# sp-uhh/sgmse

Measured on AMD Instinct MI355X. Metric: utterances/sec, SGMSE+ NCSN++ PC N=30 (reverse_diffusion + ALD, 60 NFE), 16 kHz 4 s utterances, higher is better.
Workload: dtype f32 (fp16x2-split products, fp32 accumulate); 1 GPU; BASELINE configs[1]: ncsnpp (65.6M params) PC sampler N=30, batch=32 x 4 s @16 kHz per GPU, hipGraph-captured step; batch_per_gpu=32, F=256, T=512, nfe=60, sampler=pc, parallelism=utterance-sharded x1 (weights broadcast once over RCCL)

## Files before the change

### sgmse_amd/csrc/conv_launch.h

```cpp
#pragma once
#include "kernels_conv.h"
#include "kernels_conv_pipe.h"
#include "kernels_conv1x1.h"
#include "kernels_conv_split.h"
#include "kernels_conv_wino.h"
#include "kernels_conv_wino2d.h"
#include "kernels_conv_thin.h"

#ifndef SGMSE_CONV_SPLIT_DEFAULT
#define SGMSE_CONV_SPLIT_DEFAULT 2
#endif
#ifndef SGMSE_CONV_PIPE_DEFAULT
#define SGMSE_CONV_PIPE_DEFAULT 1
#endif

namespace sgmse {

inline int conv_variant() {
  static int v = [] { const char* e = getenv("SGMSE_CONV_VARIANT"); return e ? atoi(e) : 0; }();
  return v;
}

inline int conv_grid_tiles(const ConvArgs& a, int rows) {
  const int ty = (a.H + rows - 1) / rows;
  return a.rag_cols ? ty * a.rag_ncols : a.B * ty * ((a.W + 31) / 32);
}

template <int KS, int WC, int FC, int FP>
inline void launch_conv_mfma_t(const ConvArgs& a, drt::stream_t st, int variant, int ksplit = 1) {
  using T = ConvTile<KS, WC, FC, FP>;
  const int tiles = conv_grid_tiles(a, T::ROWS);
  dim3 grid(tiles, (a.Cout + T::CO_T - 1) / T::CO_T, ksplit);
  if (variant < 0) variant = conv_variant();
  const bool vec = (a.rag_w ? a.rag_vec_ok != 0 : a.W % 4 == 0) && !(variant & 2) && (reinterpret_cast<uintptr_t>(a.src1) % 16 == 0) &&
                   (a.src2 == nullptr || reinterpret_cast<uintptr_t>(a.src2) % 16 == 0);
  const bool pref = !(variant & 1);
  if constexpr (FC * FP == 8) {
    const bool pipe = ((variant & 4) != 0) != (SGMSE_CONV_PIPE_DEFAULT != 0);
    if (vec && pipe) { DRT_LAUNCH((conv_mfma_pipe_kernel<KS, WC, FC, FP>), grid, dim3(256), st, a); return; }
  }
  if constexpr (KS == 1 && FC * FP == 8) {
    if (!vec) { launch_conv_mfma_t<KS, WC, FC, FP / 2>(a, st, variant, ksplit); return; }
    if (pref) DRT_LAUNCH((conv_mfma_kernel<KS, WC, FC, FP, 1, 1>), grid, dim3(256), st, a);
    else DRT_LAUNCH((conv_mfma_kernel<KS, WC, FC, FP, 0, 1>), grid, dim3(256), st, a);
  } else {
    if (vec && pref) DRT_LAUNCH((conv_mfma_kernel<KS, WC, FC, FP, 1, 1>), grid, dim3(256), st, a);
    else if (vec) DRT_LAUNCH((conv_mfma_kernel<KS, WC, FC, FP, 0, 1>), grid, dim3(256), st, a);
    else if (pref) DRT_LAUNCH((conv_mfma_kernel<KS, WC, FC, FP, 1, 0>), grid, dim3(256), st, a);
    else DRT_LAUNCH((conv_mfma_kernel<KS, WC, FC, FP, 0, 0>), grid, dim3(256), st, a);
  }
  if constexpr (FC * FP <= 2) {
    if (ksplit > 1) DRT_LAUNCH((conv_splitk_reduce_kernel<KS, WC, FC, FP>), dim3(grid.x, grid.y, 1), dim3(256), st, a, ksplit);
  }
}

inline void launch_conv_mfma(const ConvArgs& a, int ks, const ConvPlan& pl, drt::stream_t st, int variant = -1, int ksplit = 1) {
  const int v = variant < 0 ? conv_variant() : variant;
  if (ks == 1 && pl.co_t == 128 && (v & 8)) {
    const int kc = (v & 16) ? 64 : 32;
    const int Cin = a.C1 + a.C2;
    if (Cin % kc == 0 && (a.src2 == nullptr || a.C1 % kc == 0)) {
      const int tiles = conv_grid_tiles(a, 4);
      dim3 grid(tiles, a.Cout / 128, 1);
      if (kc == 64) DRT_LAUNCH((conv1x1_stream_kernel<1, 64>), grid, dim3(256), st, a);
      else DRT_LAUNCH((conv1x1_stream_kernel<1, 32>), grid, dim3(256), st, a);
      return;
    }
  }
#define SGMSE_CONV_CASE(KS_, CO_, ROWS_, WC_, FC_, FP_) \
  if (ks == KS_ && pl.co_t == CO_ && pl.rows == ROWS_) { launch_conv_mfma_t<KS_, WC_, FC_, FP_>(a, st, variant, ksplit); return; }
  SGMSE_CONV_CASE(3, 128, 8, 2, 2, 4)
  SGMSE_CONV_CASE(3, 64, 8, 2, 1, 4)
  SGMSE_CONV_CASE(3, 32, 8, 1, 1, 2)
  SGMSE_CONV_CASE(3, 128, 4, 2, 2, 2)
  SGMSE_CONV_CASE(3, 64, 4, 2, 1, 2)
  SGMSE_CONV_CASE(3, 32, 4, 1, 1, 1)
  SGMSE_CONV_CASE(1, 128, 8, 2, 2, 4)
  SGMSE_CONV_CASE(1, 64, 8, 2, 1, 4)
  SGMSE_CONV_CASE(1, 32, 8, 1, 1, 2)
  SGMSE_CONV_CASE(1, 128, 4, 2, 2, 2)
  SGMSE_CONV_CASE(1, 64, 4, 2, 1, 2)
  SGMSE_CONV_CASE(1, 32, 4, 1, 1, 1)
#undef SGMSE_CONV_CASE
}

inline bool conv_split_eligible(int ks, int C1, int C2, int Cout) {
  return (ks == 3 || ks == 1) && Cout % 128 == 0 && (C1 + C2) % 16 == 0 && (C2 == 0 || C1 % 16 == 0) && (C1 + C2) <= 512;
}
inline bool conv_thin_split_eligible(int ks, int C1, int C2, int Cout) {
  return ks == 3 && Cout <= 32 && (C1 + C2) >= 64 && (C1 + C2) % 16 == 0 && (C2 == 0 || C1 % 16 == 0) && (C1 + C2) <= 512;
}
template <class S, int SHAPE>
inline void launch_conv3x3_split_t(const ConvArgs& a, dim3 grid, drt::stream_t st) {
  const bool act = a.in_scale && a.in_act;
  if constexpr (SHAPE != 1 && S::SCALED) {
    if (a.sc_w) {
      DRT_LAUNCH((conv3x3_split_kernel<S, SHAPE, 1, 0, 1>), grid, dim3(256), st, a);
      return;
    }
  }
  if (act) DRT_LAUNCH((conv3x3_split_kernel<S, SHAPE, 1>), grid, dim3(256), st, a);
  else DRT_LAUNCH((conv3x3_split_kernel<S, SHAPE, 0>), grid, dim3(256), st, a);
}
inline int conv_split_stats_rows(int ks, int Cout) { return (ks == 3 && Cout <= 32) ? 1 : 4; }
inline void launch_conv_split(const ConvArgs& a, int ks, int mode, drt::stream_t st, bool rows4 = false, int abl = 0, int ksplit = 1) {
  const int tiles = conv_grid_tiles(a, 8);
  if (ks == 3 && a.Cout > 32 && rows4 && a.kchunk_stages > 0 && mode == 2) {
    const dim3 grid(conv_grid_tiles(a, 4), a.Cout / 128, ksplit);
    if (a.in_scale && a.in_act) DRT_LAUNCH((conv3x3_split_kernel<SplitH2, 2, 1, 0, 0, 1>), grid, dim3(256), st, a);
    else DRT_LAUNCH((conv3x3_split_kernel<SplitH2, 2, 0, 0, 0, 1>), grid, dim3(256), st, a);
    if (ksplit > 1) DRT_LAUNCH((conv_splitk_reduce_kernel<3, 4, 1, 4, true>), dim3(grid.x, grid.y, 1), dim3(256), st, a, ksplit);
    return;
  }
  if (ks == 3 && a.Cout > 32 && rows4) {
    const dim3 grid(conv_grid_tiles(a, 4), a.Cout / 128, 1);
    if (mode == 2) launch_conv3x3_split_t<SplitH2, 2>(a, grid, st); else launch_conv3x3_split_t<SplitB3, 2>(a, grid, st);
    return;
  }
  if (ks == 3 && a.Cout <= 32) {
    if (mode == 2) launch_conv3x3_split_t<SplitH2, 1>(a, dim3(tiles, 1, 1), st); else launch_conv3x3_split_t<SplitB3, 1>(a, dim3(tiles, 1, 1), st);
    return;
  }
  if (ks == 1) {
    if (mode == 2) DRT_LAUNCH(conv1x1_split_kernel<SplitH2>, dim3(tiles, a.Cout / 128, 1), dim3(256), st, a);
    else DRT_LAUNCH(conv1x1_split_kernel<SplitB3>, dim3(tiles, a.Cout / 128, 1), dim3(256), st, a);
    return;
  }
  const dim3 grid(tiles, a.Cout / 128, 1);
  if (abl && mode == 2) {
#define SGMSE_ABL_CASE(V) if (abl == V) { DRT_LAUNCH((conv3x3_split_kernel<SplitH2, 0, 1, V>), grid, dim3(256), st, a); return; }
#ifdef SGMSE_ABLATION_FULL
    SGMSE_ABL_CASE(8) SGMSE_ABL_CASE(59) SGMSE_ABL_CASE(64)
    SGMSE_ABL_CASE(3) SGMSE_ABL_CASE(4) SGMSE_ABL_CASE(24) SGMSE_ABL_CASE(56)
    SGMSE_ABL_CASE(1) SGMSE_ABL_CASE(2) SGMSE_ABL_CASE(67) SGMSE_ABL_CASE(72) SGMSE_ABL_CASE(128) SGMSE_ABL_CASE(256) SGMSE_ABL_CASE(512)
#endif
#undef SGMSE_ABL_CASE
  }
  if (mode == 2) launch_conv3x3_split_t<SplitH2, 0>(a, grid, st); else launch_conv3x3_split_t<SplitB3, 0>(a, grid, st);
}

inline bool conv_wino_eligible(int C1, int C2, int Cout, int W) {
  return Cout % 128 == 0 && (C1 + C2) % 16 == 0 && (C2 == 0 || C1 % 16 == 0) && (C1 + C2) <= 512 && W % 2 == 0;
}
inline void launch_conv_wino(const ConvArgs& a, drt::stream_t st, bool rows4, bool trace = false, int abl = 0) {
  const bool act = a.in_scale && a.in_act;
#ifdef SGMSE_ABLATION_FULL
#define SGMSE_WABL_CASE(V) if (abl == V) { DRT_LAUNCH((conv3x3_wino_kernel<8, 1, 0, 0, V>), dim3(conv_grid_tiles(a, 8), a.Cout / 128, 1), dim3(512), st, a); return; }
  SGMSE_WABL_CASE(1) SGMSE_WABL_CASE(2) SGMSE_WABL_CASE(4) SGMSE_WABL_CASE(8) SGMSE_WABL_CASE(16) SGMSE_WABL_CASE(24) SGMSE_WABL_CASE(3) SGMSE_WABL_CASE(32) SGMSE_WABL_CASE(20)
#undef SGMSE_WABL_CASE
  if (trace) { DRT_LAUNCH((conv3x3_wino_kernel<8, 1, 0, 1>), dim3(conv_grid_tiles(a, 8), a.Cout / 128, 1), dim3(512), st, a); return; }
#endif
  (void)abl; (void)trace;
  if (rows4) {
    const dim3 grid(conv_grid_tiles(a, 4), a.Cout / 128, 1);
    if (a.sc_w) DRT_LAUNCH((conv3x3_wino_kernel<4, 1, 1>), grid, dim3(512), st, a);
    else if (act) DRT_LAUNCH((conv3x3_wino_kernel<4, 1, 0>), grid, dim3(512), st, a);
    else DRT_LAUNCH((conv3x3_wino_kernel<4, 0, 0>), grid, dim3(512), st, a);
  } else {
    const dim3 grid(conv_grid_tiles(a, 8), a.Cout / 128, 1);
    if (a.sc_w) DRT_LAUNCH((conv3x3_wino_kernel<8, 1, 1>), grid, dim3(512), st, a);
    else if (act) DRT_LAUNCH((conv3x3_wino_kernel<8, 1, 0>), grid, dim3(512), st, a);
    else DRT_LAUNCH((conv3x3_wino_kernel<8, 0, 0>), grid, dim3(512), st, a);
  }
}

inline void launch_conv_wino2d(const ConvArgs& a, drt::stream_t st, int abl = 0) {
  const dim3 grid(conv_grid_tiles(a, 4), a.Cout / 128, 1);
  const bool act = a.in_scale && a.in_act;
  if (abl == 8) { DRT_LAUNCH((conv3x3_wino2d_kernel<1, 8>), grid, dim3(512), st, a); return; }
  if (abl == 16) { DRT_LAUNCH((conv3x3_wino2d_kernel<1, 16>), grid, dim3(512), st, a); return; }
  if (act) DRT_LAUNCH((conv3x3_wino2d_kernel<1>), grid, dim3(512), st, a);
  else DRT_LAUNCH((conv3x3_wino2d_kernel<0>), grid, dim3(512), st, a);
}

inline void launch_conv_thin(const ConvArgs& a, drt::stream_t st) {
  const dim3 grid(conv_thin_grid_tiles(a, (a.W + ConvThinGeom::TW - 1) / ConvThinGeom::TW), 1, 1);
  if (a.in_scale && a.in_act) DRT_LAUNCH((conv3x3_thin_kernel<1>), grid, dim3(256), st, a);
  else DRT_LAUNCH((conv3x3_thin_kernel<0>), grid, dim3(256), st, a);
}

inline void launch_conv_direct(const ConvArgs& a, int ks, drt::stream_t st) {
  const int HW = a.H * a.W;
  if (a.Cout <= 4) {
    dim3 grid((HW + 255) / 256, 1, a.B);
    if (ks == 3) DRT_LAUNCH((conv_direct_kernel<3, 4>), grid, dim3(256), st, a);
    else DRT_LAUNCH((conv_direct_kernel<1, 4>), grid, dim3(256), st, a);
  } else {
    dim3 grid((HW + 255) / 256, (a.Cout + 15) / 16, a.B);
    if (ks == 3) DRT_LAUNCH((conv_direct_kernel<3, 16>), grid, dim3(256), st, a);
    else DRT_LAUNCH((conv_direct_kernel<1, 16>), grid, dim3(256), st, a);
  }
}

}
```

### sgmse_amd/csrc/engine.h

```cpp
#pragma once
#include <map>
#include <string>
#include <vector>
#include <cstdio>
#include <stdexcept>

#include <deque>
#include <sgmse_devrt.h>
#include "kernels_conv.h"
#include "conv_launch.h"
#include "kernels_norm_fir.h"
#include "kernels_attn_misc.h"
#include "kernels_stft.h"

namespace sgmse {

struct EngineError : std::runtime_error { using std::runtime_error::runtime_error; };

#define SG_CHECK(expr) do { int _e = (expr); if (_e != 0) { char _b[256]; snprintf(_b, sizeof _b, "%s failed: %s (%d)", #expr, drt::error_string(_e), _e); throw EngineError(_b); } } while (0)
#define SG_REQUIRE(cond, msg) do { if (!(cond)) throw EngineError(std::string(msg)); } while (0)

struct NetCfg {
  int variant = 0;
  int nf = 128;
  int n_levels = 7;
  int ch_mult[8] = {1, 1, 2, 2, 2, 2, 2, 0};
  int num_res_blocks = 2;
  int n_attn = 1;
  int attn_res[8] = {16, 0, 0, 0, 0, 0, 0, 0};
  int image_size = 256;
  int progressive = 1;
  int progressive_input = 1;
  int scale_by_sigma = 1;
};

struct Mod {
  enum Kind { FOURIER, LINEAR, CONV3, RES, ATTN, COMBINE, GN } kind;
  int idx, cin, cout;
  bool up, down;
};

inline bool cfg_has_attn(const NetCfg& c, int res) {
  for (int i = 0; i < c.n_attn; ++i) if (c.attn_res[i] == res) return true;
  return false;
}

inline std::vector<Mod> build_layout(const NetCfg& c) {
  std::vector<Mod> mods;
  auto add = [&](Mod::Kind k, int cin, int cout, bool up = false, bool down = false) {
    mods.push_back(Mod{k, (int)mods.size(), cin, cout, up, down});
  };
  const int nf = c.nf, L = c.n_levels, temb = 4 * nf, channels = 4;
  add(Mod::FOURIER, 0, nf);
  add(Mod::LINEAR, 2 * nf, temb);
  add(Mod::LINEAR, temb, temb);
  add(Mod::CONV3, channels, nf);
  std::vector<int> hs_c{nf};
  int in_ch = nf;
  for (int l = 0; l < L; ++l) {
    const int res = c.image_size >> l;
    for (int r = 0; r < c.num_res_blocks; ++r) {
      const int out_ch = nf * c.ch_mult[l];
      add(Mod::RES, in_ch, out_ch);
      in_ch = out_ch;
      if (cfg_has_attn(c, res)) add(Mod::ATTN, in_ch, in_ch);
      hs_c.push_back(in_ch);
    }
    if (l != L - 1) {
      add(Mod::RES, in_ch, in_ch, false, true);
      if (c.progressive_input == 1) add(Mod::COMBINE, channels, in_ch);
      hs_c.push_back(in_ch);
    }
  }
  in_ch = hs_c.back();
  add(Mod::RES, in_ch, in_ch);
  add(Mod::ATTN, in_ch, in_ch);
  add(Mod::RES, in_ch, in_ch);
  for (int l = L - 1; l >= 0; --l) {
    const int res = c.image_size >> l;
    for (int r = 0; r < c.num_res_blocks + 1; ++r) {
      const int out_ch = nf * c.ch_mult[l];
      const int cin = in_ch + hs_c.back();
      hs_c.pop_back();
      add(Mod::RES, cin, out_ch);
      in_ch = out_ch;
    }
    if (cfg_has_attn(c, res)) add(Mod::ATTN, in_ch, in_ch);
    if (c.progressive == 1) { add(Mod::GN, in_ch, in_ch); add(Mod::CONV3, in_ch, channels); }
    if (l != 0) add(Mod::RES, in_ch, in_ch, true, false);
  }
  SG_REQUIRE(hs_c.empty(), "layout: skip stack not empty");
  if (c.progressive != 1) { add(Mod::GN, in_ch, in_ch); add(Mod::CONV3, in_ch, channels); }
  return mods;
}

inline std::vector<std::pair<std::string, size_t>> param_manifest(const NetCfg& c) {
  std::vector<std::pair<std::string, size_t>> out;
  out.push_back({"output_layer.weight", 8});
  out.push_back({"output_layer.bias", 2});
  const int temb = 4 * c.nf;
  for (const Mod& m : build_layout(c)) {
    const std::string p = "all_modules." + std::to_string(m.idx) + ".";
    auto put = [&](const char* k, size_t n) { out.push_back({p + k, n}); };
    switch (m.kind) {
      case Mod::FOURIER: put("W", c.nf); break;
      case Mod::LINEAR: put("weight", (size_t)m.cout * m.cin); put("bias", m.cout); break;
      case Mod::CONV3: put("weight", (size_t)m.cout * m.cin * 9); put("bias", m.cout); break;
      case Mod::GN: put("weight", m.cin); put("bias", m.cin); break;
      case Mod::COMBINE: put("Conv_0.weight", (size_t)m.cout * m.cin); put("Conv_0.bias", m.cout); break;
      case Mod::ATTN:
        put("GroupNorm_0.weight", m.cin); put("GroupNorm_0.bias", m.cin);
        for (int i = 0; i < 4; ++i) {
          out.push_back({p + "NIN_" + std::to_string(i) + ".W", (size_t)m.cin * m.cin});
          out.push_back({p + "NIN_" + std::to_string(i) + ".b", (size_t)m.cin});
        }
        break;
      case Mod::RES:
        put("GroupNorm_0.weight", m.cin); put("GroupNorm_0.bias", m.cin);
        put("Conv_0.weight", (size_t)m.cout * m.cin * 9); put("Conv_0.bias", m.cout);
        put("Dense_0.weight", (size_t)m.cout * temb); put("Dense_0.bias", m.cout);
        put("GroupNorm_1.weight", m.cout); put("GroupNorm_1.bias", m.cout);
        put("Conv_1.weight", (size_t)m.cout * m.cout * 9); put("Conv_1.bias", m.cout);
        if (m.cin != m.cout || m.up || m.down) { put("Conv_2.weight", (size_t)m.cout * m.cin); put("Conv_2.bias", m.cout); }
        break;
    }
  }
  return out;
}

struct PackArgs { const float* src[3]; int nsrc, cout_per_src, io, cin, taps, cout, co_t; float* dst; size_t total; };

__global__ __launch_bounds__(256) void pack_weights_kernel(PackArgs p) {
  const size_t e = (size_t)blockIdx.x * 256 + threadIdx.x;
  if (e >= p.total) return;
  const int j = (int)(e % p.co_t);
  size_t r = e / p.co_t;
  const int t = (int)(r % p.taps); r /= p.taps;
  const int c = (int)(r % p.cin);
  const int blk = (int)(r / p.cin);
  const int co = blk * p.co_t + j;
  float v = 0.f;
  if (co < p.cout) {
    const int s = co / p.cout_per_src, cj = co % p.cout_per_src;
    v = p.io ? p.src[s][(size_t)c * p.cout_per_src + cj] : p.src[s][((size_t)cj * p.cin + c) * p.taps + t];
  }
  p.dst[e] = v;
}

__global__ __launch_bounds__(256) void pad_cin_kernel(const float* src, float* dst, int cout, int cin, int cin_pad, int taps) {
  const size_t e = (size_t)blockIdx.x * 256 + threadIdx.x;
  if (e >= (size_t)cout * cin_pad * taps) return;
  const int t = (int)(e % taps);
  const int c = (int)((e / taps) % cin_pad);
  const int co = (int)(e / ((size_t)taps * cin_pad));
  dst[e] = c < cin ? src[((size_t)co * cin + c) * taps + t] : 0.f;
}

__global__ __launch_bounds__(256) void zero_floats_kernel(float* p, int n) {
  const int i = blockIdx.x * 256 + threadIdx.x;
  if (i < n) p[i] = 0.f;
}

__global__ __launch_bounds__(256) void fill_random_kernel(float* dst, size_t n, uint32_t seed) {
  const size_t i = (size_t)blockIdx.x * 256 + threadIdx.x;
  if (i >= n) return;
  uint32_t h = (uint32_t)i * 2654435761u ^ seed;
  h ^= h >> 16; h *= 0x7feb352du; h ^= h >> 15; h *= 0x846ca68bu; h ^= h >> 16;
  dst[i] = (float)(h >> 8) * (2.0f / 16777216.0f) - 1.0f;
}

template <int VEC, int WRITE>
__global__ __launch_bounds__(256) void calib_stream_kernel(float* buf, size_t nvec, float* sink) {
  struct alignas(VEC * 4) vec_t { float v[VEC]; };
  vec_t* p = reinterpret_cast<vec_t*>(buf);
  const size_t per = (nvec + gridDim.x - 1) / gridDim.x;
  const size_t lo = (size_t)blockIdx.x * per, hi = lo + per < nvec ? lo + per : nvec;
  float acc = 0.f;
  for (size_t i = lo + threadIdx.x; i < hi; i += 256) {
    if constexpr (WRITE) { vec_t v; for (int k = 0; k < VEC; ++k) v.v[k] = (float)(i & 1023); p[i] = v; }
    else { const vec_t v = p[i]; for (int k = 0; k < VEC; ++k) acc += v.v[k]; }
  }
  if (!WRITE && acc == 123456.789f) sink[0] = acc;
}

__global__ __launch_bounds__(256) void lds_poison_kernel(unsigned* sink, unsigned salt) {
  __shared__ unsigned s[40960];
  for (int i = threadIdx.x; i < 40960; i += 256) s[i] = 0x7FC00000u | ((unsigned)i + salt);
  __syncthreads();
  if (s[(threadIdx.x * 97 + salt) % 40960] == 0x12345678u) sink[0] = 1u;
}

__global__ __launch_bounds__(256) void transpose_io_kernel(const float* src, float* dst, int cin, int cout) {
  const int e = blockIdx.x * 256 + threadIdx.x;
  if (e >= cin * cout) return;
  const int co = e / cin, c = e % cin;
  dst[e] = src[(size_t)c * cout + co];
}

class Arena {
 public:
  void reset() { free_.clear(); free_.push_back({0, cap_}); live_.clear(); deferring_ = false; deferred_.clear(); }
  void configure(char* base, size_t cap) { base_ = base; cap_ = cap; live_.clear(); reset(); }
  void measure_mode() { base_ = reinterpret_cast<char*>(uintptr_t(1) << 44); cap_ = size_t(1) << 42; high_ = 0; reset(); live_.clear(); }
  size_t high_water() const { return high_; }
  float* alloc(size_t nfloats) {
    size_t bytes = (nfloats * 4 + 255) / 256 * 256;
    if (bytes == 0) bytes = 256;
    for (size_t i = 0; i < free_.size(); ++i) {
      if (free_[i].second >= bytes) {
        const size_t off = free_[i].first;
        free_[i].first += bytes; free_[i].second -= bytes;
        if (free_[i].second == 0) free_.erase(free_.begin() + i);
        live_[off] = bytes;
        if (off + bytes > high_) high_ = off + bytes;
        return reinterpret_cast<float*>(base_ + off);
      }
    }
    throw EngineError("activation arena exhausted");
  }
  void defer_begin() { deferring_ = true; }
  void defer_end() { deferring_ = false; std::vector<float*> d; d.swap(deferred_); for (float* p : d) release(p); }
  void release(float* p) {
    if (!p) return;
    if (deferring_) { deferred_.push_back(p); return; }
    const size_t off = size_t(reinterpret_cast<char*>(p) - base_);
    auto it = live_.find(off);
    SG_REQUIRE(it != live_.end(), "arena: bad release");
    size_t bytes = it->second;
    live_.erase(it);
    size_t i = 0;
    while (i < free_.size() && free_[i].first < off) ++i;
    free_.insert(free_.begin() + i, {off, bytes});
    if (i + 1 < free_.size() && free_[i].first + free_[i].second == free_[i + 1].first) {
      free_[i].second += free_[i + 1].second; free_.erase(free_.begin() + i + 1);
    }
    if (i > 0 && free_[i - 1].first + free_[i - 1].second == free_[i].first) {
      free_[i - 1].second += free_[i].second; free_.erase(free_.begin() + i);
    }
  }
 private:
  char* base_ = nullptr;
  size_t cap_ = 0, high_ = 0;
  std::vector<std::pair<size_t, size_t>> free_;
  std::map<size_t, size_t> live_;
  bool deferring_ = false;
  std::vector<float*> deferred_;
};

struct Tensor { float* p = nullptr; int C = 0, H = 0, W = 0; float* st = nullptr; int nsub = 0; float* amax = nullptr; int srows = 1; };

struct ConvW {
  const float* oihw = nullptr;
  const float* packed = nullptr;
  const float* packed32 = nullptr;
  const float* packed_thin = nullptr;
  const float* packed_split = nullptr;
  const float* split_scale = nullptr;
  int split_mode = 0;
  const float* packed_wino = nullptr;
  const float* wino_scale = nullptr;
  const float* bias = nullptr;
  int ks = 1, cin = 0, cout = 0, co_t = 0;
};

struct ResW { const float *g0w, *g0b, *g1w, *g1b; ConvW c0, c1, c2; bool has_c2; int temb_off; };
struct AttnW { const float *gw, *gb; ConvW qkv, proj; };

struct SamplerCfg {
  int N = 30;
  int corrector = 1;
  float snr = 0.f;
  int corrector_steps = 1;
  int predictor = 1;
  int probability_flow = 0;
  int denoise = 1;
  float theta = 1.5f;
  float std1 = 0.f;
  const float* t = nullptr; const float* dt = nullptr; const float* ald_eps = nullptr; const float* ald_noise = nullptr;
  const float* G = nullptr; const float* G2 = nullptr;
  const float* in_scale = nullptr; const float* score_alpha = nullptr; const float* score_beta = nullptr;
  int use_graph = 1;
};

class Engine {
 public:
  explicit Engine(int device, void* stream) : device_(device) {
    SG_CHECK(drt::set_device(device));
    stream_ = reinterpret_cast<drt::stream_t>(stream);
    read_knobs();
  }
  ~Engine() {
    for (void* p : owned_) drt::free_dev(p);
    for (void* p : wowned_) drt::free_dev(p);
    if (graph_valid_ || graph_stale_) drt::graph_destroy(&graph_);
    if (hstage_) drt::free_host(hstage_);
    if (hstage_ev_init_) drt::event_destroy(&hstage_ev_);
    for (drt::event_t& e : side_ev_) drt::event_destroy(&e);
    if (side_stream_ready_) drt::stream_destroy(side_stream_);
    for (ProfRec& r : prof_recs_) { drt::event_destroy(&r.a); drt::event_destroy(&r.b); }
  }

  drt::stream_t stream() const { return stream_; }
  void set_stream(void* s) { stream_ = reinterpret_cast<drt::stream_t>(s); }

  void set_config(const NetCfg& c) { cfg_ = c; layout_ = build_layout(c); weights_ready_ = false; invalidate_graph(); read_knobs(); }
  const NetCfg& config() const { return cfg_; }

  void load_weights(const char* const* names, const void* const* ptrs, const long long* numels, int n, int on_device) {
    invalidate_graph();
    weights_ready_ = false;
    free_weight_allocs();
    auto manifest = param_manifest(cfg_);
    std::map<std::string, size_t> want;
    size_t total = 0;
    for (auto& kv : manifest) { want[kv.first] = kv.second; total += (kv.second + 63) / 64 * 64; }
    float* blob = static_cast<float*>(dev_alloc_w(total * 4));
    blob_ = blob; blob_elems_ = total;
    std::map<std::string, std::pair<const void*, long long>> given;
    for (int i = 0; i < n; ++i) given[names[i]] = {ptrs[i], numels[i]};
    size_t off = 0;
    W_.clear();
    for (auto& kv : manifest) {
      auto it = given.find(kv.first);
      if (it == given.end()) throw EngineError("load_weights: missing parameter " + kv.first);
      if ((size_t)it->second.second != kv.second)
        throw EngineError("load_weights: size mismatch for " + kv.first + " (got " + std::to_string(it->second.second) +
                          ", want " + std::to_string(kv.second) + ")");
      if (on_device) SG_CHECK(drt::memcpy_d2d(blob + off, it->second.first, kv.second * 4, stream_));
      else SG_CHECK(drt::memcpy_h2d(blob + off, it->second.first, kv.second * 4, stream_));
      W_[kv.first] = blob + off;
      off += (kv.second + 63) / 64 * 64;
    }
    if (!on_device) SG_CHECK(drt::stream_sync(stream_));
    read_knobs();
    finalize_weights();
  }

  size_t param_count() const { size_t n = 0; for (auto& kv : param_manifest(cfg_)) n += kv.second; return n; }

  struct FwdCtl {
    const float* bias_table; int bias_bstride, bias_sstride; const int* step_ptr;
    const float* tvals; int t_bstride, t_sstride; float sign;
    const float* coef = nullptr; int coef_bstride = 0, coef_sstride = 0;
    const int* bias_step = nullptr;
    int y_plane = 0;
  };

  void forward_xy(const float2* xy, const float* t_dev, float2* out, int B, int F, int T) {
    require_ready();
    ensure_shape(B, F, T, B);
    compute_temb(t_dev, B);
    FwdCtl ctl{bias_table_, tot_temb_, 0, nullptr, t_dev, 1, 0, 1.0f};
    const long long FT = (long long)F * T;
    arena_.reset();
    if (ragged()) {
      ctl.y_plane = 1;
      run_forward(xy, 2, xy, 2, out, B, F, T, ctl);
    } else {
      run_forward(xy, 2 * FT, xy + FT, 2 * FT, out, B, F, T, ctl);
    }
  }

  void pc_sample(const float2* Y, float2* out, int B, int F, int T, const SamplerCfg& sc, const float2* noise,
                 unsigned long long seed) {
    require_ready();
    SG_REQUIRE(sc.N >= 1 && sc.t && sc.dt && sc.G && sc.G2, "pc_sample: step table missing");
    SG_REQUIRE(sc.corrector != 1 || (sc.ald_eps && sc.ald_noise), "pc_sample: ALD table missing");
    ensure_shape(B, F, T, sc.N);
    SG_REQUIRE(!ragged() || sc.corrector != 2, "ragged batches: the Langevin corrector couples the utterances of a batch (correctors.py:50-52) and is not supported");
    SG_REQUIRE(!ragged() || !noise, "ragged batches: replayed noise is not supported (in-kernel noise only)");
    const size_t n = ragged() ? rag_pix_[0] : (size_t)B * F * T;
    std::vector<float> tab((size_t)sc.N * SC_STRIDE, 0.f), tv(sc.N);
    for (int i = 0; i < sc.N; ++i) {
      float* r = &tab[(size_t)i * SC_STRIDE];
      r[SC_T] = sc.t[i]; r[SC_DT] = sc.dt[i]; r[SC_G] = sc.G[i]; r[SC_G2] = sc.G2[i];
      if (sc.corrector == 1) { r[SC_ALD_EPS] = sc.ald_eps[i]; r[SC_ALD_NOISE] = sc.ald_noise[i]; }
      tv[i] = sc.t[i];
    }
    const bool affine = sc.in_scale && sc.score_alpha && sc.score_beta;
    SG_REQUIRE(affine || (!sc.in_scale && !sc.score_alpha && !sc.score_beta), "pc_sample: give all three score-wrapper arrays or none");
    std::vector<float> cf;
    if (affine) {
      cf.assign((size_t)sc.N * 4, 0.f);
      for (int i = 0; i < sc.N; ++i) { cf[4 * i] = sc.in_scale[i]; cf[4 * i + 1] = sc.score_alpha[i]; cf[4 * i + 2] = sc.score_beta[i]; }
    }
    const unsigned long long* seed_dev = upload_tables(tab, tv, cf, seed, B);
    compute_temb(tsteps_, sc.N);

    const int ncorr = sc.corrector ? sc.corrector_steps : 0;
    const bool pred_noise = sc.predictor == 1 && !sc.probability_flow;
    const int draws_per_step = ncorr + (pred_noise ? 1 : 0);

    SG_CHECK(drt::memcpy_d2d(sy_, Y, n * 8, stream_));
    Y = sy_;
    SamplerArgs sa{};
    sa.x = sx_; sa.x_mean = sxm_; sa.y = Y; sa.score = sscore_; sa.noise = noise; sa.seed = seed_dev;
    sa.table = step_table_; sa.step_ptr = step_ctr_; sa.theta = sc.theta; sa.std1 = sc.std1; sa.n = (int)n;
    sa.score_w = sc.probability_flow ? 0.5f : 1.0f;
    sa.snr = sc.snr; sa.B = B; sa.per = F * T; sa.partial = lang_partial_; sa.lang = lang_scal_;
    sa.rag_off = ragged() ? rag_off_dev_[0] : nullptr;
    const dim3 eg((unsigned)((n + 255) / 256));

    sa.draw_base = 0; sa.draw_per_step = 0;
    DRT_LAUNCH(sampler_prior_kernel, eg, dim3(256), stream_, sa);
    SG_CHECK(drt::memcpy_d2d(sxm_, sx_, n * 8, stream_));
    DRT_LAUNCH(step_set_kernel, dim3(1), dim3(64), stream_, step_ctr_, 0);

    FwdCtl ctl{bias_table_, 0, tot_temb_, step_ctr_, tsteps_, 0, 1, -1.0f};
    if (affine) { ctl.coef = coef_table_; ctl.coef_bstride = 0; ctl.coef_sstride = 1; }
    const long long FT = ragged() ? 1 : (long long)F * T;
    auto step_body = [&]() {
      for (int cs = 0; cs < ncorr; ++cs) {
        arena_.reset();
        run_forward(sx_, FT, Y, FT, sscore_, B, F, T, ctl);
        SamplerArgs a = sa; a.draw_base = 1 + cs; a.draw_per_step = draws_per_step;
        if (sc.corrector == 2) {
          DRT_LAUNCH(sampler_langevin_norms_kernel, dim3(LANG_NBLK, B), dim3(256), stream_, a);
          DRT_LAUNCH(sampler_langevin_scalars_kernel, dim3(1), dim3(64), stream_, a);
          DRT_LAUNCH(sampler_langevin_kernel, eg, dim3(256), stream_, a);
        } else {
          DRT_LAUNCH(sampler_ald_kernel, eg, dim3(256), stream_, a);
        }
      }
      if (sc.predictor == 1) {
        arena_.reset();
        run_forward(sx_, FT, Y, FT, sscore_, B, F, T, ctl);
        SamplerArgs a = sa; a.draw_base = 1 + ncorr; a.draw_per_step = draws_per_step; a.add_noise = pred_noise ? 1 : 0;
        DRT_LAUNCH(sampler_revdiff_kernel, eg, dim3(256), stream_, a);
      }
      if (sc.predictor == 0 && ncorr > 0) SG_CHECK(drt::memcpy_d2d(sxm_, sx_, n * 8, stream_));
      DRT_LAUNCH(step_inc_kernel, dim3(1), dim3(64), stream_, step_ctr_);
    };

    GraphKey key{B, F, T, sc.corrector, ncorr, sc.predictor, sc.probability_flow + (affine ? 2 : 0), (const void*)Y, (const void*)noise,
                 sc.theta + 1000.f * sc.snr * (sc.corrector == 2), draws_per_step};
    const bool want_graph = sc.use_graph && drt::graphs_supported();
    if (want_graph) {
      if (!graph_valid_ || !(key == graph_key_)) {
        invalidate_graph();
        capture_step(step_body);
        graph_key_ = key;
      }
      for (int i = 0; i < sc.N; ++i) SG_CHECK(drt::graph_launch(&graph_, stream_));
    } else {
      for (int i = 0; i < sc.N; ++i) step_body();
    }
    SG_CHECK(drt::memcpy_d2d(out, sc.denoise ? sxm_ : sx_, n * 8, stream_));
    nfe_ = sc.N * (ncorr + 1);
  }
  void sb_sample(const float2* Y, float2* out, int B, int F, int T, int N, const float* t, const float* w_prev, const float* w_est,
                 const float* w_y, const float* w_z, const float* in_scale, const float* alpha, const float* beta, int stochastic,
                 const float2* noise, unsigned long long seed, int use_graph) {
    require_ready();
    SG_REQUIRE(N >= 1 && t && w_prev && w_est && w_y && w_z, "sb_sample: step table missing");
    SG_REQUIRE(!ragged(), "ragged batches: not supported by the Schroedinger-bridge sampler");
    ensure_shape(B, F, T, N);
    const size_t n = (size_t)B * F * T;
    std::vector<float> tab((size_t)N * SC_STRIDE, 0.f), tv(N);
    for (int i = 0; i < N; ++i) {
      float* r = &tab[(size_t)i * SC_STRIDE];
      r[SC_T] = t[i]; r[SB_WPREV] = w_prev[i]; r[SB_WEST] = w_est[i]; r[SB_WY] = w_y[i]; r[SB_WZ] = w_z[i];
      tv[i] = t[i];
    }
    const bool affine = in_scale && alpha && beta;
    SG_REQUIRE(affine || (!in_scale && !alpha && !beta), "sb_sample: give all three score-wrapper arrays or none");
    std::vector<float> cf;
    if (affine) {
      cf.assign((size_t)N * 4, 0.f);
      for (int i = 0; i < N; ++i) { cf[4 * i] = in_scale[i]; cf[4 * i + 1] = alpha[i]; cf[4 * i + 2] = beta[i]; }
    }
    const unsigned long long* seed_dev = upload_tables(tab, tv, cf, seed, B);
    compute_temb(tsteps_, N);
    SG_CHECK(drt::memcpy_d2d(sy_, Y, n * 8, stream_));
    SG_CHECK(drt::memcpy_d2d(sx_, Y, n * 8, stream_));
    DRT_LAUNCH(step_set_kernel, dim3(1), dim3(64), stream_, step_ctr_, 0);

    SamplerArgs sa{};
    sa.x = sx_; sa.x_mean = sxm_; sa.y = sy_; sa.score = sscore_; sa.noise = noise; sa.seed = seed_dev;
    sa.table = step_table_; sa.step_ptr = step_ctr_; sa.n = (int)n; sa.add_noise = stochastic ? 1 : 0; sa.B = B; sa.per = F * T;
    sa.draw_base = 0; sa.draw_per_step = 1;
    const dim3 eg((unsigned)((n + 255) / 256));
    FwdCtl ctl{bias_table_, 0, tot_temb_, step_ctr_, tsteps_, 0, 1, -1.0f};
    if (affine) { ctl.coef = coef_table_; ctl.coef_bstride = 0; ctl.coef_sstride = 1; }
    const long long FT = (long long)F * T;
    auto step_body = [&]() {
      arena_.reset();
      run_forward(sx_, FT, sy_, FT, sscore_, B, F, T, ctl);
      DRT_LAUNCH(sampler_sb_kernel, eg, dim3(256), stream_, sa);
      DRT_LAUNCH(step_inc_kernel, dim3(1), dim3(64), stream_, step_ctr_);
    };
    GraphKey key{B, F, T, 100 + stochastic, 0, 0, affine ? 2 : 0, nullptr, (const void*)noise, 0.f, 1};
    if (use_graph && drt::graphs_supported()) {
      if (!graph_valid_ || !(key == graph_key_)) {
        invalidate_graph();
        capture_step(step_body);
        graph_key_ = key;
      }
      for (int i = 0; i < N; ++i) SG_CHECK(drt::graph_launch(&graph_, stream_));
    } else {
      for (int i = 0; i < N; ++i) step_body();
    }
    SG_CHECK(drt::memcpy_d2d(out, sx_, n * 8, stream_));
    nfe_ = N;
  }
  void set_noise_streams(const unsigned long long* ids, int n) { streams_next_.assign(ids, ids + n); }
  void set_ragged_frames(const int* frames, int n) { set_frames(frames, n); }
  int last_nfe() const { return nfe_; }
  int graph_captures() const { return graph_captures_; }
  int graph_updates() const { return graph_updates_; }
  int split_mode() const { return split_mode_; }
  bool winograd() const { return split_mode_ == 2 && wino_; }
  size_t arena_bytes() const { return arena_cap_; }

  float* input_bounds(const float* x1, int C1, const float* x2, int C2, int B, int HW) {
    const size_t per = (size_t)B * kAmaxSpread;
    float* out = static_cast<float*>(dev_alloc_tmp(2 * per * 4));
    SG_CHECK(drt::memset_dev(out, 0, 2 * per * 4, stream_));
    for (int b = 0; b < B; ++b) {
      const size_t n1 = (size_t)C1 * HW;
      DRT_LAUNCH(absmax_kernel, dim3((unsigned)std::min<size_t>((n1 + 255) / 256, 1024)), dim3(256), stream_, x1 + b * n1, n1,
                 out + (size_t)b * kAmaxSpread);
      if (x2) {
        const size_t n2 = (size_t)C2 * HW;
        DRT_LAUNCH(absmax_kernel, dim3((unsigned)std::min<size_t>((n2 + 255) / 256, 1024)), dim3(256), stream_, x2 + b * n2, n2,
                   out + per + (size_t)b * kAmaxSpread);
      }
    }
    return out;
  }

  float* producer_bound(const float* in_scale, const float* in_shift, int C, const float* amax1, const float* amax2, int B) {
    float* out = static_cast<float*>(dev_alloc_tmp((size_t)B * kAmaxSpread * 4));
    DRT_LAUNCH(xform_bound_kernel, dim3(B), dim3(64), stream_, in_scale, in_shift, C, amax1, amax2, out);
    return out;
  }

  void op_conv2d(const float* x, const float* w_oihw, const float* bias, const float* res, float* out, int B, int Cin,
                 int Cout, int H, int W, int ks, float out_scale, int force_direct, const float* in_scale,
                 const float* in_shift, int in_act, const float* x2, int C2) {
    ConvArgs a{};
    a.src1 = x; a.src2 = x2; a.C1 = Cin - C2; a.C2 = C2; a.bias = bias; a.res = res; a.out_scale = out_scale; a.out = out;
    a.Cout = Cout; a.B = B; a.H = H; a.W = W; a.in_scale = in_scale; a.in_shift = in_shift; a.in_act = in_act;
    ConvPlan pl = choose_conv_plan(ks, Cin, Cout, H, W);
    if (force_direct == 6) {
      SG_REQUIRE(conv_thin_eligible(ks, a.C1, C2, Cout), "op_conv2d: shape is not eligible for the thin-output kernel");
      const float* pk = pack_thin(w_oihw, Cin, Cout, false);
      a.w = pk;
      launch_conv_thin(a, stream_);
      SG_CHECK(drt::stream_sync(stream_));
      free_tmp(const_cast<float*>(pk));
    } else if (force_direct == 7) {
      SG_REQUIRE(ks == 3 && conv_wino_eligible(a.C1, C2, Cout, W), "op_conv2d: shape is not eligible for the 2-D Winograd kernel");
      const float* pk = pack_wino2d(w_oihw, Cin, Cout, false, &a.co_scale);
      a.w = pk;
      float* bounds = input_bounds(x, a.C1, x2, C2, B, H * W);
      const float* am2 = x2 ? bounds + (size_t)B * kAmaxSpread : nullptr;
      float* xb = producer_bound(in_scale, in_shift, Cin, bounds, am2, B);
      a.xbound = xb;
      launch_conv_wino2d(a, stream_);
      SG_CHECK(drt::stream_sync(stream_));
      free_tmp(const_cast<float*>(pk)); free_tmp(bounds); free_tmp(xb);
    } else if (force_direct == 4 || force_direct == 5) {
      SG_REQUIRE(ks == 3 && conv_wino_eligible(a.C1, C2, Cout, W), "op_conv2d: shape is not eligible for the Winograd kernel");
      const float* pk = pack_wino(w_oihw, Cin, Cout, false, &a.co_scale);
      a.w = pk;
      float* bounds = input_bounds(x, a.C1, x2, C2, B, H * W);
      const float* am2 = x2 ? bounds + (size_t)B * kAmaxSpread : nullptr;
      float* xb = producer_bound(in_scale, in_shift, Cin, bounds, am2, B);
      a.xbound = xb;
      launch_conv_wino(a, stream_, force_direct == 5);
      SG_CHECK(drt::stream_sync(stream_));
      free_tmp(const_cast<float*>(pk)); free_tmp(bounds); free_tmp(xb);
    } else if (force_direct == 2 || force_direct == 3) {
      SG_REQUIRE(conv_split_eligible(ks, a.C1, C2, Cout) || conv_thin_split_eligible(ks, a.C1, C2, Cout),
                 "op_conv2d: shape is not eligible for the split kernels");
      const int smode = force_direct - 1;
      const float* pk = pack_split(w_oihw, ks, Cin, Cout, smode, false, &a.co_scale);
      a.w = pk;
      float *bounds = nullptr, *xb = nullptr;
      if (smode == 2) {
        SG_REQUIRE(ks == 3 || in_scale == nullptr, "op_conv2d: the fp16x2 1x1 kernel takes raw inputs (no fused producer)");
        bounds = input_bounds(x, a.C1, x2, C2, B, H * W);
        const float* am2 = x2 ? bounds + (size_t)B * kAmaxSpread : nullptr;
        if (ks == 1) { a.amax1 = bounds; a.amax2 = am2; }
        else { xb = producer_bound(in_scale, in_shift, Cin, bounds, am2, B); a.xbound = xb; }
      }
      launch_conv_split(a, ks, smode, stream_);
      SG_CHECK(drt::stream_sync(stream_));
      free_tmp(const_cast<float*>(pk));
      if (bounds) free_tmp(bounds);
      if (xb) free_tmp(xb);
    } else if (pl.mfma && !force_direct && (C2 == 0 || a.C1 % ((ks == 3) ? 8 : 32) == 0)) {
      const size_t ne = packed_weight_elems(ks, Cin, Cout, pl.co_t);
      float* pk = static_cast<float*>(dev_alloc_tmp(ne * 4));
      PackArgs pa{}; pa.src[0] = w_oihw; pa.nsrc = 1; pa.cout_per_src = Cout; pa.io = 0; pa.cin = Cin; pa.taps = ks * ks;
      pa.cout = Cout; pa.co_t = pl.co_t; pa.dst = pk; pa.total = ne;
      DRT_LAUNCH(pack_weights_kernel, dim3((unsigned)((ne + 255) / 256)), dim3(256), stream_, pa);
      a.w = pk;
      launch_conv_mfma(a, ks, pl, stream_);
      SG_CHECK(drt::stream_sync(stream_));
      free_tmp(pk);
    } else {
      a.w = w_oihw;
      launch_conv_direct(a, ks, stream_);
    }
    check_launch();
  }

  void op_groupnorm(const float* x, const float* gamma, const float* beta, float* out, int B, int C, int H, int W, int act,
                    const float* x2, int C2) {
    const int HW = H * W, C1 = C - C2;
    float* stats = static_cast<float*>(dev_alloc_tmp((size_t)B * C * 2 * 4));
    float* sc = static_cast<float*>(dev_alloc_tmp((size_t)B * C * 4));
    float* sh = static_cast<float*>(dev_alloc_tmp((size_t)B * C * 4));
    float* stats2 = stats + (size_t)B * C1 * 2;
    DRT_LAUNCH(gn_chan_stats_kernel, dim3(B * C1), dim3(256), stream_, x, (const float*)nullptr, C1, 0, HW, stats, Rag{nullptr, nullptr, nullptr}, 0);
    if (C2) DRT_LAUNCH(gn_chan_stats_kernel, dim3(B * C2), dim3(256), stream_, x2, (const float*)nullptr, C2, 0, HW, stats2, Rag{nullptr, nullptr, nullptr}, 0);
    const int G = std::min(C / 4, 32);
    const GnFin f{stats, stats2, nullptr, nullptr, gamma, beta, sc, sh, nullptr, Rag{nullptr, nullptr, nullptr}, C1, 1, 1, C2, 1, 1, G, HW, 0, 1e-6f};
    DRT_LAUNCH(gn_finalize_kernel, dim3(G, B), dim3(256), stream_, f);
    DRT_LAUNCH(gn_apply_kernel, dim3((HW + 1023) / 1024, B * C), dim3(256), stream_, x, x2, C1, C2, HW, (const float*)sc,
               (const float*)sh, act, out);
    SG_CHECK(drt::stream_sync(stream_));
    check_launch();
    free_tmp(stats); free_tmp(sc); free_tmp(sh);
  }

  void op_fir(const float* x, float* out, int BC, int H, int W, int up, const float* in_scale, const float* in_shift, int in_act,
              float* out_raw) {
    FirArgs fa{x, out, in_scale, in_shift, in_act, BC, H, W, out_raw, 1, Rag{nullptr, nullptr, nullptr}};
    launch_fir(fa, up);
    check_launch();
  }

  void op_upfirdn2d(int dtype, const void* x, const void* kern, void* out, int BC, int H, int W, int kh, int kw, int up_x, int up_y,
                    int down_x, int down_y, int px0, int px1, int py0, int py1) {
    UpfirdnArgs a{x, kern, out, BC, H, W, kh, kw, up_x, up_y, down_x, down_y, px0, px1, py0, py1, 0, 0};
    a.Ho = (H * up_y + py0 + py1 - kh) / down_y + 1;
    a.Wo = (W * up_x + px0 + px1 - kw) / down_x + 1;
    SG_REQUIRE(a.Ho > 0 && a.Wo > 0, "upfirdn2d: empty output");
    const dim3 grid((a.Ho * a.Wo + 255) / 256, BC);
    if (dtype == 0) DRT_LAUNCH(upfirdn2d_generic_kernel<UpfirdnF32>, grid, dim3(256), stream_, a);
    else if (dtype == 1) DRT_LAUNCH(upfirdn2d_generic_kernel<UpfirdnF64>, grid, dim3(256), stream_, a);
    else DRT_LAUNCH(upfirdn2d_generic_kernel<UpfirdnF16>, grid, dim3(256), stream_, a);
    check_launch();
  }

  void op_attention(const float* qkv, float* out, int B, int C, int S) {
    AttnArgs a{qkv, out, B, C, S, 1.0f / sqrtf((float)C), Rag{nullptr, nullptr, nullptr}, 0};
    SG_REQUIRE(launch_attn_core(a, stream_), "attention: C must be 32, 64, 128 or 256");
    check_launch();
  }

  void op_stft(const float* sig, const float* window, float2* spec, int B, int L, int n_fft, int hop) {
    SG_REQUIRE(n_fft <= kMaxNfft && n_fft >= 2 && hop >= 1 && L > n_fft / 2, "stft: unsupported geometry");
    const float2* tw = twiddle(n_fft);
    StftArgs a{sig, window, tw, spec, L, n_fft, hop, n_fft / 2 + 1, (L + 2 * (n_fft / 2) - n_fft) / hop + 1};
    DRT_LAUNCH(stft_kernel, dim3(a.K, B), dim3(256), stream_, a);
    check_launch();
  }

  void op_istft(const float2* spec, const float* window, float* out, int B, int K, int n_fft, int hop, int length) {
    SG_REQUIRE(n_fft <= kMaxNfft && n_fft >= 2 && hop >= 1, "istft: unsupported geometry");
    SG_REQUIRE(K >= 1 && length >= 1 && length + n_fft / 2 <= n_fft + hop * (K - 1), "istft: length exceeds the overlap-add span");
    const float2* tw = twiddle(n_fft);
    IstftArgs a{spec, window, tw, out, n_fft, hop, n_fft / 2 + 1, K, length};
    DRT_LAUNCH(istft_kernel, dim3((length + 255) / 256, B), dim3(256), stream_, a);
    check_launch();
  }

  void op_spec_xform(const float2* in, float2* out, size_t n, int type, float factor, float exponent, int inverse) {
    SpecXformArgs a{in, out, n, type, factor, exponent, inverse};
    DRT_LAUNCH(spec_xform_kernel, dim3((unsigned)((n + 255) / 256)), dim3(256), stream_, a);
    check_launch();
  }

  void sync() { SG_CHECK(drt::stream_sync(stream_)); }

  float bench_conv(int ks, int B, int Cin, int Cout, int H, int W, int variant, int iters, int fused) {
    ConvPlan pl = choose_conv_plan(ks, Cin, Cout, H, W);
    SG_REQUIRE(pl.mfma, "bench_conv: shape is not MFMA-eligible");
    if (variant >= 0 && (variant & 512)) { pl.rows = 4; variant &= ~512; }
    int ablate = 0, abl_split = 0;
    bool split_rows4 = false;
    if (variant >= 0) {
      split_rows4 = (variant >> 23) & 1;
      abl_split = (variant >> 12) & 1023;
      if (!(variant & (64 | 128))) { ablate = abl_split & 15; abl_split = 0; }
      variant &= 4095;
    }
    const bool wino = variant >= 0 && (variant & 1024);
    const bool wino2d = variant >= 0 && (variant & 2048) && !wino;
    const int smode = variant < 0 ? 0 : ((variant & 128) ? 2 : ((variant & 64) ? 1 : 0));
    const bool b3 = smode != 0 && !wino && !wino2d;
    SG_REQUIRE(!(wino || wino2d) || (ks == 3 && conv_wino_eligible(Cin, 0, Cout, W)), "bench_conv: shape is not eligible for the Winograd kernel");
    SG_REQUIRE(!b3 || conv_split_eligible(ks, Cin, 0, Cout), "bench_conv: shape is not eligible for the split kernels");
    const size_t nx = (size_t)B * Cin * H * W, no = (size_t)B * Cout * H * W, nw = (size_t)Cout * Cin * ks * ks;
    const size_t ne = packed_weight_elems(ks, Cin, Cout, pl.co_t);
    float* x = static_cast<float*>(dev_alloc_tmp(nx * 4));
    float* o = static_cast<float*>(dev_alloc_tmp(no * 4));
    float* r = static_cast<float*>(dev_alloc_tmp(no * 4));
    float* w = static_cast<float*>(dev_alloc_tmp(nw * 4));
    float* pk = static_cast<float*>(dev_alloc_tmp(ne * 4));
    float* sc = static_cast<float*>(dev_alloc_tmp((size_t)B * Cin * 8));
    auto fill = [&](float* d, size_t n, uint32_t seed) {
      DRT_LAUNCH(fill_random_kernel, dim3((unsigned)((n + 255) / 256)), dim3(256), stream_, d, n, seed);
    };
    fill(x, nx, 1); fill(r, no, 2); fill(w, nw, 3); fill(sc, (size_t)B * Cin * 2, 4);
    PackArgs pa{}; pa.src[0] = w; pa.nsrc = 1; pa.cout_per_src = Cout; pa.io = 0; pa.cin = Cin; pa.taps = ks * ks; pa.cout = Cout;
    pa.co_t = pl.co_t; pa.dst = pk; pa.total = ne;
    DRT_LAUNCH(pack_weights_kernel, dim3((unsigned)((ne + 255) / 256)), dim3(256), stream_, pa);
    ConvArgs a{};
    a.src1 = x; a.C1 = Cin; a.w = pk; a.out = o; a.Cout = Cout; a.B = B; a.H = H; a.W = W; a.out_scale = 1.f;
    a.ablate = ablate;
    if (fused) { a.in_scale = sc; a.in_shift = sc + (size_t)B * Cin; a.in_act = 1; a.res = r; a.bias = w; a.out_scale = 0.70710678f; }
    drt::event_t e0{}, e1{};
    drt::event_create(&e0); drt::event_create(&e1);
    const float* pk3 = nullptr;
    float *bounds = nullptr, *xbound = nullptr;
    if (b3) {
      pk3 = pack_split(w, ks, Cin, Cout, smode, false, &a.co_scale); a.w = pk3;
      if (smode == 2) {
        bounds = input_bounds(x, Cin, nullptr, 0, B, H * W);
        if (ks == 1) {
          a.in_scale = nullptr; a.in_shift = nullptr; a.in_act = 0;
          a.amax1 = bounds;
        } else {
          xbound = producer_bound(a.in_scale, a.in_shift, Cin, bounds, nullptr, B); a.xbound = xbound;
        }
      }
    }
    if (wino || wino2d) {
      pk3 = wino2d ? pack_wino2d(w, Cin, Cout, false, &a.co_scale) : pack_wino(w, Cin, Cout, false, &a.co_scale); a.w = pk3;
      bounds = input_bounds(x, Cin, nullptr, 0, B, H * W);
      xbound = producer_bound(a.in_scale, a.in_shift, Cin, bounds, nullptr, B); a.xbound = xbound;
    }
    unsigned long long* trace_dev = nullptr;
    const size_t n_wg = (size_t)B * ((H + 7) / 8) * ((W + 31) / 32) * ((Cout + 127) / 128);
    if (abl_split & 64) {
      trace_dev = static_cast<unsigned long long*>(dev_alloc_tmp(n_wg * 256));
      SG_CHECK(drt::memset_dev(trace_dev, 0, n_wg * 256, stream_));
      a.trace = trace_dev;
    }
    auto go = [&]() {
      if (wino2d) launch_conv_wino2d(a, stream_, abl_split & 63);
      else if (wino) launch_conv_wino(a, stream_, split_rows4, (abl_split & 64) != 0, abl_split & 63);
      else if (b3) launch_conv_split(a, ks, smode, stream_, split_rows4, abl_split);
      else launch_conv_mfma(a, ks, pl, stream_, variant);
    };
    for (int i = 0; i < 2; ++i) go();
    drt::event_record(&e0, stream_);
    for (int i = 0; i < iters; ++i) go();
    drt::event_record(&e1, stream_);
    drt::event_sync(&e1);
    const float ms = drt::event_elapsed_ms(e0, e1) / (float)iters;
    check_launch();
    drt::event_destroy(&e0); drt::event_destroy(&e1);
    if (trace_dev) {
      const size_t words = wino ? 32 : 16;
      std::vector<unsigned long long> h(n_wg * words);
      SG_CHECK(drt::memcpy_d2h(h.data(), trace_dev, n_wg * words * 8, stream_));
      SG_CHECK(drt::stream_sync(stream_));
      if (const char* path = getenv("SGMSE_TRACE_OUT")) { if (FILE* f = fopen(path, "wb")) { fwrite(h.data(), 8, h.size(), f); fclose(f); } }
      free_tmp(trace_dev);
    }
    for (float* q : {x, o, r, w, pk, sc}) free_tmp(q);
    if (pk3) free_tmp(const_cast<float*>(pk3));
    if (bounds) free_tmp(bounds);
    if (xbound) free_tmp(xbound);
    return ms;
  }

  float calib_stream(int mode, int bytes_per_lane, size_t total_bytes) {
    SG_REQUIRE((bytes_per_lane == 8 || bytes_per_lane == 16) && (mode == 0 || mode == 1) && total_bytes >= 4096, "calib_stream: bad arguments");
    float* buf = static_cast<float*>(dev_alloc_tmp(total_bytes + 256));
    SG_CHECK(drt::memset_dev(buf, 0, total_bytes + 256, stream_));
    const size_t nvec = total_bytes / (size_t)bytes_per_lane;
    drt::event_t e0{}, e1{};
    drt::event_create(&e0); drt::event_create(&e1);
    drt::event_record(&e0, stream_);
    const dim3 g(256 * 16), b(256);
    float* sink = buf + total_bytes / 4;
    if (bytes_per_lane == 8) { if (mode) DRT_LAUNCH((calib_stream_kernel<2, 1>), g, b, stream_, buf, nvec, sink); else DRT_LAUNCH((calib_stream_kernel<2, 0>), g, b, stream_, buf, nvec, sink); }
    else { if (mode) DRT_LAUNCH((calib_stream_kernel<4, 1>), g, b, stream_, buf, nvec, sink); else DRT_LAUNCH((calib_stream_kernel<4, 0>), g, b, stream_, buf, nvec, sink); }
    drt::event_record(&e1, stream_);
    drt::event_sync(&e1);
    const float ms = drt::event_elapsed_ms(e0, e1);
    check_launch();
    drt::event_destroy(&e0); drt::event_destroy(&e1);
    free_tmp(buf);
    return ms;
  }

  enum { TC_CONV3_BIG = 0, TC_CONV3, TC_CONV1, TC_DIRECT, TC_GN, TC_FIR, TC_ATTN, TC_MISC, TC_COUNT };
  void profile_forward(const float2* xy, const float* t_dev, float2* out, int B, int F, int T, float* ms_out, double* work_out,
                       int* launches_out) {
    prof_ = true;
    for (int i = 0; i < TC_COUNT; ++i) { prof_ms_[i] = 0.f; prof_flops_[i] = 0.0; prof_n_[i] = 0; }
    prof_used_ = 0;
    forward_xy(xy, t_dev, out, B, F, T);
    prof_ = false;
    SG_CHECK(drt::stream_sync(stream_));
    for (size_t i = 0; i < prof_used_; ++i) {
      ProfRec& r = prof_recs_[i];
      if (r.cls < 0) continue;
      const float ms = drt::event_elapsed_ms(r.a, r.b);
      prof_ms_[r.cls] += ms;
      prof_flops_[r.cls] += r.work;
      prof_n_[r.cls] += r.launches;
      if (prof_dump_ && r.note[0]) fprintf(stderr, "[sgmse-prof] %s %.4f ms %.1f Gwork/s\n", r.note, ms, r.work / ms * 1e-6);
    }
    for (int i = 0; i < TC_COUNT; ++i) { ms_out[i] = prof_ms_[i]; work_out[i] = prof_flops_[i]; launches_out[i] = prof_n_[i]; }
  }

 private:
  void* dev_alloc_w(size_t bytes) {
    void* p = nullptr;
    SG_CHECK(drt::malloc_dev(&p, bytes ? bytes : 256));
    if (poison_) SG_CHECK(drt::memset_dev(p, 0xFF, bytes ? bytes : 256, stream_));
    wowned_.push_back(p);
    return p;
  }
  void free_weight_allocs() {
    if (wowned_.empty()) return;
    drt::stream_sync(stream_);
    for (void* p : wowned_) drt::free_dev(p);
    wowned_.clear();
  }
  void* dev_alloc(size_t bytes) {
    void* p = nullptr;
    SG_CHECK(drt::malloc_dev(&p, bytes ? bytes : 256));
    if (poison_) SG_CHECK(drt::memset_dev(p, 0xFF, bytes ? bytes : 256, stream_));
    owned_.push_back(p);
    return p;
  }
  void* dev_alloc_tmp(size_t bytes) {
    void* p = nullptr;
    SG_CHECK(drt::malloc_dev(&p, bytes ? bytes : 256));
    if (poison_) SG_CHECK(drt::memset_dev(p, 0xFF, bytes ? bytes : 256, stream_));
    return p;
  }
  void free_tmp(void* p) { drt::free_dev(p); }
  void dev_free_owned(void* p) {
    for (size_t i = 0; i < owned_.size(); ++i) if (owned_[i] == p) { owned_.erase(owned_.begin() + i); break; }
    drt::free_dev(p);
  }
  void check_launch() { SG_CHECK(drt::last_error()); }
  void require_ready() { SG_REQUIRE(weights_ready_, "weights not loaded (call sgmse_load_weights first)"); }
  void invalidate_graph() { if (graph_valid_) { graph_valid_ = false; graph_stale_ = true; } }
  void drop_graph() { if (graph_valid_ || graph_stale_) { drt::graph_destroy(&graph_); graph_valid_ = graph_stale_ = false; } }
  template <class Body>
  void capture_step(Body&& body) {
    SG_CHECK(drt::stream_sync(stream_));
    SG_CHECK(drt::graph_begin_capture(stream_));
    capturing_ = true;
    try { body(); } catch (...) {
      capturing_ = false;
      drt::graph_abort_capture(stream_);
      drop_graph();
      throw;
    }
    capturing_ = false;
    if (graph_stale_) {
      const int r = drt::graph_end_capture_update(stream_, &graph_);
      if (r > 0) { drt::graph_destroy(&graph_); graph_stale_ = false; graph_valid_ = false; SG_CHECK(r); }
      if (r == 0) ++graph_updates_; else ++graph_captures_;
    } else {
      const int r = drt::graph_end_capture(stream_, &graph_);
      if (r != 0) { drt::graph_destroy(&graph_); graph_valid_ = false; SG_CHECK(r); }
      ++graph_captures_;
    }
    graph_stale_ = false;
    graph_valid_ = true;
  }
  bool graph_stale_ = false, capturing_ = false; int graph_updates_ = 0;

  const float2* twiddle(int n_fft) {
    auto it = twiddles_.find(n_fft);
    if (it != twiddles_.end()) return it->second;
    std::vector<float2> h(n_fft);
    for (int m = 0; m < n_fft; ++m) {
      const double ang = 2.0 * 3.14159265358979323846 * (double)m / (double)n_fft;
      h[m] = make_float2((float)cos(ang), (float)sin(ang));
    }
    float2* d = static_cast<float2*>(dev_alloc(sizeof(float2) * n_fft));
    SG_CHECK(drt::memcpy_h2d(d, h.data(), sizeof(float2) * n_fft, stream_));
    SG_CHECK(drt::stream_sync(stream_));
    twiddles_[n_fft] = d;
    return d;
  }

  const float* Wp(const std::string& name) const {
    auto it = W_.find(name);
    if (it == W_.end()) throw EngineError("internal: unknown parameter " + name);
    return it->second;
  }

  ConvW make_conv(const std::string& wname, const std::string& bname, int ks, int cin, int cout) {
    return make_conv(Wp(wname), bname.empty() ? nullptr : Wp(bname), ks, cin, cout);
  }
  ConvW make_conv(const float* oihw, const float* bias, int ks, int cin, int cout) {
    ConvW c; c.ks = ks; c.cin = cin; c.cout = cout;
    c.oihw = oihw; c.bias = bias;
    ConvPlan pl = choose_conv_plan(ks, cin, cout, 8, 32);
    if (pl.mfma) {
      c.co_t = pl.co_t;
      const size_t ne = packed_weight_elems(ks, cin, cout, pl.co_t);
      float* pk = static_cast<float*>(dev_alloc_w(ne * 4));
      PackArgs pa{}; pa.src[0] = c.oihw; pa.nsrc = 1; pa.cout_per_src = cout; pa.io = 0; pa.cin = cin; pa.taps = ks * ks;
      pa.cout = cout; pa.co_t = pl.co_t; pa.dst = pk; pa.total = ne;
      DRT_LAUNCH(pack_weights_kernel, dim3((unsigned)((ne + 255) / 256)), dim3(256), stream_, pa);
      c.packed = pk;
      if (pl.co_t > 32) {
        const size_t ne32 = packed_weight_elems(ks, cin, cout, 32);
        float* pk32 = static_cast<float*>(dev_alloc_w(ne32 * 4));
        PackArgs pb = pa; pb.co_t = 32; pb.dst = pk32; pb.total = ne32;
        DRT_LAUNCH(pack_weights_kernel, dim3((unsigned)((ne32 + 255) / 256)), dim3(256), stream_, pb);
        c.packed32 = pk32;
      }
    }
    if (split_mode_ && (conv_split_eligible(ks, cin, 0, cout) || conv_thin_split_eligible(ks, cin, 0, cout))) {
      c.split_mode = split_mode_;
      c.packed_split = pack_split(c.oihw, ks, cin, cout, c.split_mode, true, &c.split_scale);
    }
    if (conv_thin_eligible(ks, cin, 0, cout)) c.packed_thin = pack_thin(c.oihw, cin, cout, true);
    if (split_mode_ == 2 && wino_ && ks == 3 && conv_wino_eligible(cin, 0, cout, 2)) c.packed_wino = pack_wino(c.oihw, cin, cout, true, &c.wino_scale);
    return c;
  }

  const float* pack_split(const float* oihw, int ks, int cin, int cout, int mode, bool weight_owned, const float** scale_out) {
    const int taps = ks * ks;
    const size_t frags = mode == 2 ? packed_split_frags<SplitH2>(cin, cout, taps) : packed_split_frags<SplitB3>(cin, cout, taps);
    const int cout_pad = (cout + 127) / 128 * 128;
    const size_t bytes = frags * 16 + (size_t)cout_pad * 8;
    uint32_t* pk = static_cast<uint32_t*>(weight_owned ? dev_alloc_w(bytes) : dev_alloc_tmp(bytes));
    PackSplitArgs pa{oihw, pk, cin, cout, frags, nullptr, taps};
    const dim3 grid((unsigned)((frags + 255) / 256));
    if (mode == 2) {
      float* inv = reinterpret_cast<float*>(pk) + frags * 4;
      float* sc = inv + cout_pad;
      DRT_LAUNCH(split_co_scale_kernel, dim3((unsigned)((cout_pad + 255) / 256)), dim3(256), stream_, oihw, cin * taps, cout, cout_pad, inv, sc);
      pa.co_scale = sc;
      DRT_LAUNCH(pack_weights_split_kernel<SplitH2>, grid, dim3(256), stream_, pa);
      *scale_out = inv;
    } else {
      DRT_LAUNCH(pack_weights_split_kernel<SplitB3>, grid, dim3(256), stream_, pa);
      *scale_out = nullptr;
    }
    return reinterpret_cast<const float*>(pk);
  }

  const float* pack_thin(const float* oihw, int cin, int cout, bool weight_owned) {
    const size_t ne = packed_thin_elems(cin);
    float* pk = static_cast<float*>(weight_owned ? dev_alloc_w(ne * 4) : dev_alloc_tmp(ne * 4));
    DRT_LAUNCH(pack_weights_thin_kernel, dim3((unsigned)((ne + 255) / 256)), dim3(256), stream_, oihw, pk, cin, cout);
    return pk;
  }
  const float* pack_wino(const float* oihw, int cin, int cout, bool weight_owned, const float** scale_out) {
    const size_t frags = packed_wino_frags(cin, cout);
    const int cout_pad = (cout + 127) / 128 * 128;
    const size_t bytes = packed_wino_bytes(cin, cout) + (size_t)cout_pad * 4;
    uint32_t* pk = static_cast<uint32_t*>(weight_owned ? dev_alloc_w(bytes) : dev_alloc_tmp(bytes));
    float* inv = reinterpret_cast<float*>(pk) + frags * 4;
    float* sc = inv + cout_pad;
    DRT_LAUNCH(wino_co_scale_kernel, dim3((unsigned)((cout_pad + 255) / 256)), dim3(256), stream_, oihw, cin, cout, cout_pad, inv, sc);
    PackWinoArgs pa{oihw, pk, cin, cout, frags};
    DRT_LAUNCH(pack_weights_wino_kernel, dim3((unsigned)((frags + 255) / 256)), dim3(256), stream_, pa, (const float*)sc);
    *scale_out = inv;
    return reinterpret_cast<const float*>(pk);
  }

  const float* pack_wino2d(const float* oihw, int cin, int cout, bool weight_owned, const float** scale_out) {
    const size_t frags = packed_wino2d_frags(cin, cout);
    const int cout_pad = (cout + 127) / 128 * 128;
    const size_t bytes = packed_wino2d_bytes(cin, cout) + (size_t)cout_pad * 4;
    uint32_t* pk = static_cast<uint32_t*>(weight_owned ? dev_alloc_w(bytes) : dev_alloc_tmp(bytes));
    float* inv = reinterpret_cast<float*>(pk) + frags * 4;
    float* sc = inv + cout_pad;
    DRT_LAUNCH(wino2d_co_scale_kernel, dim3((unsigned)((cout_pad + 255) / 256)), dim3(256), stream_, oihw, cin, cout, cout_pad, inv, sc);
    PackWinoArgs pa{oihw, pk, cin, cout, frags};
    DRT_LAUNCH(pack_weights_wino2d_kernel, dim3((unsigned)((frags + 255) / 256)), dim3(256), stream_, pa, (const float*)sc);
    *scale_out = inv;
    return reinterpret_cast<const float*>(pk);
  }

  ConvW make_nin(const std::string& pre, const int* which, int nsrc, int C) {
    ConvW c; c.ks = 1; c.cin = C; c.cout = nsrc * C;
    float* tr = static_cast<float*>(dev_alloc_w((size_t)nsrc * C * C * 4));
    float* bb = static_cast<float*>(dev_alloc_w((size_t)nsrc * C * 4));
    for (int s = 0; s < nsrc; ++s) {
      const std::string n = pre + "NIN_" + std::to_string(which[s]);
      DRT_LAUNCH(transpose_io_kernel, dim3((C * C + 255) / 256), dim3(256), stream_, Wp(n + ".W"), tr + (size_t)s * C * C, C, C);
      SG_CHECK(drt::memcpy_d2d(bb + (size_t)s * C, Wp(n + ".b"), (size_t)C * 4, stream_));
    }
    c.oihw = tr; c.bias = bb;
    ConvPlan pl = choose_conv_plan(1, C, c.cout, 8, 32);
    if (pl.mfma) {
      c.co_t = pl.co_t;
      const size_t ne = packed_weight_elems(1, C, c.cout, pl.co_t);
      float* pk = static_cast<float*>(dev_alloc_w(ne * 4));
      PackArgs pa{}; pa.nsrc = nsrc; pa.cout_per_src = C; pa.io = 1; pa.cin = C; pa.taps = 1; pa.cout = c.cout; pa.co_t = pl.co_t;
      pa.dst = pk; pa.total = ne;
      for (int s = 0; s < nsrc; ++s) pa.src[s] = Wp(pre + "NIN_" + std::to_string(which[s]) + ".W");
      DRT_LAUNCH(pack_weights_kernel, dim3((unsigned)((ne + 255) / 256)), dim3(256), stream_, pa);
      c.packed = pk;
      if (pl.co_t > 32) {
        const size_t ne32 = packed_weight_elems(1, C, c.cout, 32);
        float* pk32 = static_cast<float*>(dev_alloc_w(ne32 * 4));
        PackArgs pb = pa; pb.co_t = 32; pb.dst = pk32; pb.total = ne32;
        DRT_LAUNCH(pack_weights_kernel, dim3((unsigned)((ne32 + 255) / 256)), dim3(256), stream_, pb);
        c.packed32 = pk32;
      }
    }
    if (split_mode_ && conv_split_eligible(1, C, 0, c.cout)) {
      c.split_mode = 1;
      c.packed_split = pack_split(c.oihw, 1, C, c.cout, 1, true, &c.split_scale);
    }
    return c;
  }

  void finalize_weights() {
    res_.clear(); attn_.clear(); conv_.clear(); gn_.clear();
    std::vector<DenseDesc> descs;
    int off = 0;
    for (const Mod& m : layout_) {
      const std::string p = "all_modules." + std::to_string(m.idx) + ".";
      if (m.kind == Mod::RES) {
        ResW r{};
        r.g0w = Wp(p + "GroupNorm_0.weight"); r.g0b = Wp(p + "GroupNorm_0.bias");
        r.g1w = Wp(p + "GroupNorm_1.weight"); r.g1b = Wp(p + "GroupNorm_1.bias");
        r.c0 = make_conv(p + "Conv_0.weight", p + "Conv_0.bias", 3, m.cin, m.cout);
        r.c1 = make_conv(p + "Conv_1.weight", p + "Conv_1.bias", 3, m.cout, m.cout);
        r.has_c2 = (m.cin != m.cout) || m.up || m.down;
        if (r.has_c2) r.c2 = make_conv(p + "Conv_2.weight", p + "Conv_2.bias", 1, m.cin, m.cout);
        r.temb_off = off;
        descs.push_back(DenseDesc{Wp(p + "Dense_0.weight"), Wp(p + "Dense_0.bias"), r.c0.bias, m.cout, off});
        off += m.cout;
        res_[m.idx] = r;
      } else if (m.kind == Mod::ATTN) {
        AttnW a{};
        a.gw = Wp(p + "GroupNorm_0.weight"); a.gb = Wp(p + "GroupNorm_0.bias");
        const int qkv[3] = {0, 1, 2}, pr[1] = {3};
        a.qkv = make_nin(p, qkv, 3, m.cin);
        a.proj = make_nin(p, pr, 1, m.cin);
        attn_[m.idx] = a;
      } else if (m.kind == Mod::CONV3) {
        conv_[m.idx] = make_conv(p + "weight", p + "bias", 3, m.cin, m.cout);
        if (m.cin == 4 && entry_mfma_) {
          constexpr int cp = 8;
          float* w8 = static_cast<float*>(dev_alloc_w((size_t)m.cout * cp * 9 * 4));
          DRT_LAUNCH(pad_cin_kernel, dim3((unsigned)(((size_t)m.cout * cp * 9 + 255) / 256)), dim3(256), stream_, Wp(p + "weight"), w8, m.cout, 4, cp, 9);
          entry8_ = make_conv(w8, Wp(p + "bias"), 3, cp, m.cout);
          entry8_idx_ = m.idx;
        }
      } else if (m.kind == Mod::COMBINE) {
        conv_[m.idx] = make_conv(p + "Conv_0.weight", p + "Conv_0.bias", 1, m.cin, m.cout);
      } else if (m.kind == Mod::GN) {
        gn_[m.idx] = {Wp(p + "weight"), Wp(p + "bias")};
      }
    }
    tot_temb_ = off;
    n_dense_ = (int)descs.size();
    dense_descs_ = static_cast<DenseDesc*>(dev_alloc_w(sizeof(DenseDesc) * descs.size()));
    SG_CHECK(drt::memcpy_h2d(dense_descs_, descs.data(), sizeof(DenseDesc) * descs.size(), stream_));
    SG_CHECK(drt::stream_sync(stream_));
    check_launch();
    weights_ready_ = true;
    shape_B_ = 0;
    temb_rows_ = 0;
  }

  void ensure_shape(int B, int F, int T, int nrows) {
    SG_REQUIRE(B >= 1 && F >= 1 && T >= 1, "bad shape");
    const int down = 1 << (cfg_.n_levels - 1);
    SG_REQUIRE(F % down == 0 && T % down == 0, "F and T must be multiples of 2^(levels-1) (pad_spec pads T to a multiple of 64)");
    if (B != shape_B_ || F != shape_F_ || T != shape_T_ || (ragged() && !rag_built_)) {
      invalidate_graph();
      cur_F_ = F;
      if (ragged()) build_rag_tables(B, F, T);
      arena_.measure_mode();
      dry_ = true;
      {
        FwdCtl ctl{nullptr, 0, 0, nullptr, nullptr, 0, 0, 1.f};
        run_forward(nullptr, 0, nullptr, 0, nullptr, B, F, T, ctl);
      }
      dry_ = false;
      const size_t need = arena_.high_water() + (1 << 20);
      if (need > arena_cap_) {
        if (arena_base_) dev_free_owned(arena_base_);
        arena_base_ = static_cast<char*>(dev_alloc(need));
        arena_cap_ = need;
      }
      arena_.configure(arena_base_, arena_cap_);
      const size_t n = (size_t)B * F * T;
      if (n > samp_n_) {
        for (float2** q : {&sx_, &sxm_, &sscore_, &sy_}) { if (*q) dev_free_owned(*q); *q = static_cast<float2*>(dev_alloc(n * 8)); }
        samp_n_ = n;
      }
      const size_t need_amax = (size_t)amax_next_ * B * kAmaxSpread;
      amax_slots_ = amax_next_;
      if (need_amax > amax_pool_floats_) {
        if (amax_pool_) dev_free_owned(amax_pool_);
        amax_pool_ = static_cast<float*>(dev_alloc(need_amax * 4));
        amax_pool_floats_ = need_amax;
      }
      if (!step_ctr_) step_ctr_ = static_cast<int*>(dev_alloc(256));
      if (!lang_scal_) lang_scal_ = static_cast<float*>(dev_alloc(256));
      if (lang_partial_) dev_free_owned(lang_partial_);
      lang_partial_ = static_cast<float*>(dev_alloc((size_t)B * LANG_NBLK * 2 * 4));
      shape_B_ = B; shape_F_ = F; shape_T_ = T;
    }
    if (nrows > temb_rows_) {
      invalidate_graph();
      if (temb_act_) { dev_free_owned(temb_act_); dev_free_owned(bias_table_); dev_free_owned(step_table_); dev_free_owned(tsteps_); dev_free_owned(coef_table_); dev_free_owned(bias_cur_); }
      temb_rows_ = std::max(nrows, 64);
      temb_act_ = static_cast<float*>(dev_alloc((size_t)temb_rows_ * 4 * cfg_.nf * 4));
      bias_table_ = static_cast<float*>(dev_alloc((size_t)temb_rows_ * std::max(tot_temb_, 1) * 4));
      bias_cur_ = static_cast<float*>(dev_alloc((size_t)std::max(tot_temb_, 1) * 4));
      step_table_ = static_cast<float*>(dev_alloc((size_t)temb_rows_ * SC_STRIDE * 4));
      tsteps_ = static_cast<float*>(dev_alloc((size_t)temb_rows_ * 4));
      coef_table_ = static_cast<float*>(dev_alloc((size_t)temb_rows_ * 16));
    }
  }

  void compute_temb(const float* t_dev, int rows) {
    TembArgs ta{t_dev, rows, Wp("all_modules.0.W"), Wp("all_modules.1.weight"), Wp("all_modules.1.bias"),
                Wp("all_modules.2.weight"), Wp("all_modules.2.bias"), cfg_.nf, temb_act_};
    SG_REQUIRE(cfg_.nf <= 256, "nf > 256 not supported by temb kernel");
    DRT_LAUNCH(temb_mlp_kernel, dim3(rows), dim3(256), stream_, ta);
    DRT_LAUNCH(temb_dense_kernel, dim3(n_dense_, rows), dim3(256), stream_, (const DenseDesc*)dense_descs_,
               (const float*)temb_act_, 4 * cfg_.nf, bias_table_, tot_temb_);
    check_launch();
  }

  struct Xform { const float* scale = nullptr; const float* shift = nullptr; int act = 0; const float* bound = nullptr; };

  void tick(int cls, double work, int launches = 1) {
    if (debug_sync_ && !dry_ && !capturing_) {
      const int e = drt::stream_sync(stream_);
      fprintf(stderr, "[sgmse-dbg] %s -> %s\n", prof_note_[0] ? prof_note_ : "(launch)", e ? drt::error_string(e) : "ok");
      fflush(stderr);
      if (!prof_) prof_note_[0] = 0;
    }
    if (!prof_ || prof_used_ == 0) return;
    ProfRec& r = prof_recs_[prof_used_ - 1];
    drt::event_record(&r.b, stream_);
    r.cls = cls; r.work = work; r.launches = launches;
    snprintf(r.note, sizeof r.note, "%s", prof_note_);
    prof_note_[0] = 0;
  }
  bool noting() const { return (prof_ && prof_dump_) || debug_sync_; }
  struct ProfRec { drt::event_t a{}, b{}; int cls = -1; double work = 0.0; int launches = 0; char note[160] = {0}; };
  void tock() {
    if (lds_poison_ && !dry_ && !capturing_ && !drt::is_emulator()) {
      const int idx = lds_poison_count_++;
      if (lds_poison_at_ < 0 || idx == lds_poison_at_ || (lds_poison_upto_ && idx <= lds_poison_at_)) {
        if (!lds_sink_) lds_sink_ = static_cast<unsigned*>(dev_alloc(256));
        DRT_LAUNCH(lds_poison_kernel, dim3(768), dim3(256), stream_, lds_sink_, (unsigned)idx);
      }
    }
    if (!prof_) return;
    if (prof_used_ == prof_recs_.size()) {
      prof_recs_.emplace_back();
      drt::event_create(&prof_recs_.back().a); drt::event_create(&prof_recs_.back().b);
    }
    ProfRec& r = prof_recs_[prof_used_++];
    r.cls = -1; r.note[0] = 0;
    drt::event_record(&r.a, stream_);
  }

  Tensor new_tensor(int C, int H, int W) { Tensor t; t.C = C; t.H = H; t.W = W; t.p = arena_.alloc((size_t)C * pix_total(H, W)); return t; }

  static constexpr int kNominalFrames = 512;
  bool ragged() const { return !rag_T_.empty(); }
  int level_of(int H) const { int l = 0; while ((cur_F_ >> l) > H && l < 30) ++l; return l; }
  int dec_W(int H) const { return std::max(1, kNominalFrames >> level_of(H)); }
  size_t pix_total(int H, int W) const { return ragged() ? rag_pix_.at(level_of(H)) : (size_t)B_ * H * W; }
  Rag rag_of(int H) const {
    if (!ragged()) return Rag{nullptr, nullptr, nullptr};
    const int l = level_of(H);
    return Rag{rag_w_dev_.at(l), rag_off_dev_.at(l), rag_soff_dev_.at(l)};
  }
  bool rag_all_mult2(int H) const {
    if (!ragged()) return true;
    const int l = level_of(H);
    for (int t : rag_T_) if ((t >> l) % 2) return false;
    return true;
  }
  bool rag_all_mult4(int H) const {
    if (!ragged()) return true;
    const int l = level_of(H);
    for (int t : rag_T_) if ((t >> l) % 4) return false;
    return true;
  }
  void set_frames(const int* frames, int n) {
    std::vector<int> v(frames, frames + n);
    if (v != rag_T_) { rag_T_ = v; rag_built_ = false; shape_B_ = 0; invalidate_graph(); }
  }
  void build_rag_tables(int B, int F, int T) {
    const int L = cfg_.n_levels, down = 1 << (L - 1);
    SG_REQUIRE((int)rag_T_.size() == B, "ragged batch: sgmse_set_frames gave a different number of utterances");
    int tmax = 0;
    for (int t : rag_T_) { SG_REQUIRE(t >= down && t % down == 0, "ragged batch: frame counts must be multiples of 2^(levels-1)"); tmax = std::max(tmax, t); }
    SG_REQUIRE(tmax == T, "ragged batch: T must be the largest frame count");
    for (void* q : rag_owned_) dev_free_owned(q);
    rag_owned_.clear(); rag_w_dev_.clear(); rag_off_dev_.clear(); rag_soff_dev_.clear(); rag_pix_.clear(); rag_cols_dev_.clear(); rag_ncols_.clear();
    for (int l = 0; l < L; ++l) {
      const int H = F >> l;
      std::vector<int> w(B), cols(B + 1, 0);
      std::vector<long long> off(B + 1, 0), soff(B + 1, 0);
      for (int b = 0; b < B; ++b) {
        w[b] = rag_T_[b] >> l;
        off[b + 1] = off[b] + (long long)H * w[b];
        soff[b + 1] = soff[b] + (long long)H * ((w[b] + 31) / 32);
        cols[b + 1] = cols[b] + (w[b] + 31) / 32;
      }
      int* wd = static_cast<int*>(dev_alloc((size_t)B * 4));
      long long* od = static_cast<long long*>(dev_alloc((size_t)(B + 1) * 8));
      long long* sd = static_cast<long long*>(dev_alloc((size_t)(B + 1) * 8));
      SG_CHECK(drt::memcpy_h2d(wd, w.data(), (size_t)B * 4, stream_));
      SG_CHECK(drt::memcpy_h2d(od, off.data(), (size_t)(B + 1) * 8, stream_));
      SG_CHECK(drt::memcpy_h2d(sd, soff.data(), (size_t)(B + 1) * 8, stream_));
      int* cd = static_cast<int*>(dev_alloc((size_t)(B + 1) * 4));
      SG_CHECK(drt::memcpy_h2d(cd, cols.data(), (size_t)(B + 1) * 4, stream_));
      SG_CHECK(drt::stream_sync(stream_));
      rag_owned_.push_back(cd); rag_cols_dev_.push_back(cd); rag_ncols_.push_back(cols[B]);
      rag_owned_.push_back(wd); rag_owned_.push_back(od); rag_owned_.push_back(sd);
      rag_w_dev_.push_back(wd); rag_off_dev_.push_back(od); rag_soff_dev_.push_back(sd);
      rag_pix_.push_back((size_t)off[B]);
    }
    rag_built_ = true;
  }
  std::vector<int> rag_T_;
  std::vector<int*> rag_w_dev_; std::vector<long long*> rag_off_dev_, rag_soff_dev_; std::vector<size_t> rag_pix_;
  std::vector<int*> rag_cols_dev_; std::vector<int> rag_ncols_;
  std::vector<void*> rag_owned_;
  bool rag_built_ = false;
  int cur_F_ = 0;
  void drop(Tensor& t) { arena_.release(t.p); t.p = nullptr; if (t.st) { arena_.release(t.st); t.st = nullptr; } }

  void gn_coeffs(const Tensor& a, const Tensor* b, const float* gamma, const float* beta, float** sc, float** sh,
                 const float** bound = nullptr) {
    const int C = a.C + (b ? b->C : 0), HW = a.H * a.W;
    float* bslot = bound ? next_amax() : nullptr;
    if (bound) *bound = bslot;
    const float* st[2] = {a.st, b ? b->st : nullptr};
    int nsub[2] = {a.nsub, b ? b->nsub : 0};
    int srows[2] = {a.srows, b ? b->srows : 1};
    float* tmp[2] = {nullptr, nullptr};
    const Tensor* src[2] = {&a, b};
    for (int k = 0; k < 2; ++k) {
      if (!src[k] || st[k]) continue;
      tmp[k] = arena_.alloc((size_t)B_ * src[k]->C * 2);
      st[k] = tmp[k]; nsub[k] = 1; srows[k] = 1;
      if (!dry_) {
        tock();
        DRT_LAUNCH(gn_chan_stats_kernel, dim3(B_ * src[k]->C), dim3(256), stream_, (const float*)src[k]->p, (const float*)nullptr,
                   src[k]->C, 0, HW, tmp[k], rag_of(a.H), a.H);
        if (noting()) snprintf(prof_note_, sizeof prof_note_, "gn_chan_stats C=%d @%dx%dx%d", src[k]->C, B_, a.H, a.W);
        tick(TC_GN, 4.0 * B_ * (double)src[k]->C * HW, 1);
      }
    }
    *sc = arena_.alloc((size_t)B_ * C);
    *sh = arena_.alloc((size_t)B_ * C);
    if (!dry_) {
      tock();
      const int G = std::min(C / 4, 32);
      const GnFin f{st[0], st[1], a.amax, b ? b->amax : nullptr, gamma, beta, *sc, *sh, bslot, rag_of(a.H),
                    a.C, nsub[0], srows[0], b ? b->C : 0, nsub[1], srows[1], G, HW, a.H, 1e-6f};
      DRT_LAUNCH(gn_finalize_kernel, dim3(G, B_), dim3(256), stream_, f);
      if (noting()) snprintf(prof_note_, sizeof prof_note_, "gn_finalize C=%d nsub=%d @%dx%dx%d", C, nsub[0], B_, a.H, a.W);
      tick(TC_GN, 8.0 * B_ * ((double)a.C * nsub[0] + (b ? (double)b->C * nsub[1] : 0.0)), 1);
    }
    for (int k = 0; k < 2; ++k) if (tmp[k]) arena_.release(tmp[k]);
  }

  struct Shortcut { const ConvW* w; const Tensor* a; const Tensor* b; };
  bool runs_on_h2_split3(const ConvW& w, int C, int H, int W) const {
    return w.packed && w.packed_split && w.split_mode == 2 && w.ks == 3 && w.cout > 32 && conv_split_eligible(3, C, 0, w.cout) &&
           (long)((H + 7) / 8) * ((W + 31) / 32) >= split_min_tiles_;
  }
  bool shortcut_foldable(const ConvW& c2, const Tensor& a, const Tensor* b) const {
    return fold_shortcut_ && c2.packed_split && c2.split_mode == 2 && c2.ks == 1 && conv_split_eligible(1, a.C, b ? b->C : 0, c2.cout) &&
           a.amax && (!b || b->amax);
  }

  Tensor conv(const ConvW& w, const Tensor& a, const Tensor* b, const Xform& xf, const float* bias, const float* bias2,
              const float* res, float out_scale, const FwdCtl& ctl, bool emit_stats = false, const Shortcut* sc = nullptr) {
    const int Cin = a.C + (b ? b->C : 0);
    SG_REQUIRE(Cin == w.cin, "conv: channel mismatch");
    Tensor o = new_tensor(w.cout, a.H, a.W);
    const int kc_ = (w.ks == 3) ? 8 : 32;
    const bool use_mfma = w.packed && (b == nullptr || a.C % kc_ == 0);
    int co_t = w.co_t, rows_ = a.H >= 8 ? 8 : 4;
    if (use_mfma) {
      const int cand_co[2] = {w.co_t, w.packed32 ? 32 : w.co_t};
      long best = -1;
      bool done = false;
      for (int ci = 0; ci < 2 && !done; ++ci)
        for (int rows = (a.H >= 8 ? 8 : 4); rows >= 4 && !done; rows -= 4) {
          if (ci == 1 && cand_co[1] == cand_co[0]) break;
          const long nblk = (long)B_ * ((a.H + rows - 1) / rows) * ((a.W + 31) / 32) * ((w.cout + cand_co[ci] - 1) / cand_co[ci]);
          if (nblk > best) { best = nblk; co_t = cand_co[ci]; rows_ = rows; }
          if (nblk >= tile_min_blocks_) done = true;
        }
    }
    const int Wd = dec_W(a.H);
    const long tiles8 = (long)((a.H + 7) / 8) * ((Wd + 31) / 32);
    const bool coarse_split = coarse_split_ && use_mfma && w.packed_split && w.split_mode == 2 && w.ks == 3 && w.cout > 32 && !sc &&
                              conv_split_eligible(3, a.C, b ? b->C : 0, w.cout) && tiles8 <= chunk_max_tiles_ && xf.bound != nullptr;
    const bool use_split = coarse_split || (use_mfma && w.packed_split &&
                        (conv_split_eligible(w.ks, a.C, b ? b->C : 0, w.cout) || conv_thin_split_eligible(w.ks, a.C, b ? b->C : 0, w.cout)) &&
                        tiles8 >= split_min_tiles_ &&
                        (w.split_mode != 2 || (w.ks == 3 ? xf.bound != nullptr
                                                         : (xf.scale == nullptr && a.amax && (!b || b->amax)))));
    const bool use_wino = use_split && !coarse_split && wino_ && w.packed_wino && w.ks == 3 && w.split_mode == 2 && xf.bound != nullptr &&
                          conv_wino_eligible(a.C, b ? b->C : 0, w.cout, 2) && level_of(a.H) <= 5 && tiles8 >= wino_min_tiles_;
    SG_REQUIRE(!use_wino || (a.W % 2 == 0 && (!ragged() || rag_all_mult2(a.H))), "conv: odd width on a Winograd level");
    int kchunk = 0, ksplit = 1;
    float* partial = nullptr;
    if (coarse_split) {
      const int nstages = Cin / 16;
      kchunk = std::max(2, (nstages + 7) / 8);
      const int nchunks = (nstages + kchunk - 1) / kchunk;
      const long nblk = (long)B_ * ((a.H + 3) / 4) * ((a.W + 31) / 32) * (w.cout / 128);
      if (nchunks > 1 && nblk * coarse_splitk_div_ <= tile_min_blocks_) {
        ksplit = nchunks;
        partial = arena_.alloc((size_t)nchunks * w.cout * pix_total(a.H, a.W));
      }
    }
    if (use_mfma && !use_split && coarse_chunked_ && (long)a.H * Wd <= 512 && (w.co_t == 32 || w.packed32)) {
      co_t = 32;
      const long nblk8 = (long)B_ * ((a.H + 7) / 8) * ((a.W + 31) / 32) * ((w.cout + 31) / 32);
      rows_ = (a.H >= 8 && nblk8 >= tile_min_blocks_) ? 8 : 4;
      const int nstages = Cin / kc_;
      kchunk = std::max(w.ks == 3 ? 4 : 2, (nstages + 7) / 8);
      const int nchunks = (nstages + kchunk - 1) / kchunk;
      const long nblk = (long)B_ * ((a.H + rows_ - 1) / rows_) * ((a.W + 31) / 32) * ((w.cout + 31) / 32);
      if (nchunks > 1 && nblk * 2 <= tile_min_blocks_) {
        ksplit = nchunks;
        partial = arena_.alloc((size_t)nchunks * w.cout * pix_total(a.H, a.W));
      }
    }
    if (emit_stats && use_mfma && fuse_gn_stats_) {
      o.srows = use_split ? conv_split_stats_rows(w.ks, w.cout) : 1;
      SG_REQUIRE(o.srows == 1 || !ragged() || a.H % 4 == 0, "ragged batch: 4-row statistics sub-tiles need H % 4 == 0");
      o.nsub = conv_plan_nsub(a.H, a.W, o.srows);
      o.st = arena_.alloc((size_t)B_ * w.cout * o.nsub * 2);
    } else if (emit_stats && fuse_gn_stats_) {
      o.nsub = 1;
      o.st = arena_.alloc((size_t)B_ * w.cout * 2);
    }
    o.amax = next_amax();
    if (dry_) { if (partial) arena_.release(partial); return o; }
    ConvArgs ca{};
    ca.xcd_map = conv_xcd_map_ ? 1 : 0;
    ca.stats_out = o.st; ca.stats_nsub = o.nsub; ca.stats_rows = o.srows;
    ca.amax_out = o.amax;
    ca.src1 = a.p; ca.src2 = b ? b->p : nullptr; ca.C1 = a.C; ca.C2 = b ? b->C : 0;
    ca.bias = bias; ca.bias2 = bias2; ca.bias2_bstride = ctl.bias_bstride; ca.bias2_sstride = ctl.bias_sstride;
    ca.step_ptr = bias2 ? ctl.bias_step : nullptr;
    ca.in_scale = xf.scale; ca.in_shift = xf.shift; ca.in_act = xf.act;
    ca.res = res; ca.out_scale = out_scale; ca.out = o.p; ca.Cout = w.cout; ca.B = B_; ca.H = a.H; ca.W = a.W;
    if (ragged()) {
      const Rag rg = rag_of(a.H);
      ca.rag_w = rg.w; ca.rag_off = rg.off; ca.rag_soff = rg.soff; ca.rag_slab = (long long)w.cout * (long long)pix_total(a.H, a.W);
      ca.rag_vec_ok = rag_all_mult4(a.H) ? 1 : 0;
      if (rag_prefix_) { const int l = level_of(a.H); ca.rag_cols = rag_cols_dev_.at(l); ca.rag_ncols = rag_ncols_.at(l); }
    }
    tock();
    double fl = 2.0 * B_ * (double)w.cout * Cin * w.ks * w.ks * a.H * a.W;
    if (sc) {
      SG_REQUIRE(use_split && w.ks == 3 && w.split_mode == 2 && w.cout > 32 && xf.scale && xf.act && !res, "conv: shortcut fold on an ineligible launch");
      const int Cs = sc->a->C + (sc->b ? sc->b->C : 0);
      SG_REQUIRE(Cs == sc->w->cin && sc->w->cout == w.cout && sc->a->H == a.H && sc->a->W == a.W, "conv: shortcut shape mismatch");
      ca.sc_src1 = sc->a->p; ca.sc_src2 = sc->b ? sc->b->p : nullptr; ca.sc_C1 = sc->a->C; ca.sc_C2 = sc->b ? sc->b->C : 0;
      ca.sc_w = sc->w->packed_split; ca.sc_scale = sc->w->split_scale; ca.sc_bias = sc->w->bias;
      ca.sc_amax1 = sc->a->amax; ca.sc_amax2 = sc->b ? sc->b->amax : nullptr;
      fl += 2.0 * B_ * (double)w.cout * Cs * a.H * a.W;
    }
    const bool use_thin = w.packed_thin && conv_thin_eligible(w.ks, a.C, b ? b->C : 0, w.cout) && !emit_stats && level_of(a.H) <= 1 && !bias2 && !sc;
    if (use_thin) {
      ca.w = w.packed_thin; ca.stats_out = nullptr;
      launch_conv_thin(ca, stream_);
      if (noting()) snprintf(prof_note_, sizeof prof_note_, "conv3x3-thin %d->%d @%dx%dx%d%s%s", Cin, w.cout, B_, a.H, a.W, res ? " +res" : "", xf.scale ? " +gn" : "");
      tick(TC_CONV3, fl);
      if (partial) arena_.release(partial);
    } else if (use_split) {
      ca.w = w.packed_split; ca.co_scale = w.split_scale;
      if (w.ks == 1 && w.split_mode == 2) { ca.amax1 = a.amax; ca.amax2 = b ? b->amax : nullptr; }
      if (w.ks == 3 && w.split_mode == 2) ca.xbound = xf.bound;
      const long nblk8 = (long)B_ * ((a.H + 7) / 8) * ((a.W + 31) / 32) * ((w.cout + 127) / 128);
      const bool rows4 = coarse_split || nblk8 < tile_min_blocks_;
      if (coarse_split) { ca.kchunk_stages = kchunk; ca.partial = partial; }
      if (use_wino) {
        ca.w = w.packed_wino; ca.co_scale = w.wino_scale; ca.acc_scale = nullptr;
        launch_conv_wino(ca, stream_, nblk8 < tile_min_blocks_);
      } else {
        launch_conv_split(ca, w.ks, w.split_mode, stream_, rows4, 0, ksplit);
      }
      if (coarse_split && partial) arena_.release(partial);
      if (noting()) {
        char scn[24] = "";
        if (sc) snprintf(scn, sizeof scn, " +shortcut(%d)", ca.sc_C1 + ca.sc_C2);
        snprintf(prof_note_, sizeof prof_note_, "conv3x3-%s %d->%d @%dx%dx%d%s%s%s%s", use_wino ? "wino" : "split", Cin, w.cout, B_, a.H, a.W, res ? " +res" : "",
                 xf.scale ? " +gn" : "", scn, ca.rag_cols ? " existing-tiles" : "");
      }
      tick(w.ks == 3 ? (w.cout >= 128 ? TC_CONV3_BIG : TC_CONV3) : TC_CONV1, fl);
    } else if (use_mfma) {
      ConvPlan pl{co_t, rows_, true};
      ca.w = (co_t == w.co_t) ? w.packed : w.packed32;
      ca.kchunk_stages = kchunk; ca.partial = partial;
      launch_conv_mfma(ca, w.ks, pl, stream_, -1, ksplit);
      if (partial) arena_.release(partial);
      if (noting())
        snprintf(prof_note_, sizeof prof_note_, "conv%dx%d %d->%d @%dx%dx%d tile %dco x %drows%s%s%s%s", w.ks, w.ks, Cin, w.cout, B_, a.H, a.W,
                 co_t, rows_, res ? " +res" : "", xf.scale ? " +gn" : "", ksplit > 1 ? " split-K" : "", ca.rag_cols ? " existing-tiles" : "");
      tick(w.ks == 3 ? ((split_mode_ == 0 && co_t == 128 && pl.rows == 8) ? TC_CONV3_BIG : TC_CONV3) : TC_CONV1, fl);
    } else {
      ca.w = w.oihw;
      ca.stats_out = nullptr;
      launch_conv_direct(ca, w.ks, stream_);
      if (noting()) snprintf(prof_note_, sizeof prof_note_, "conv-direct%dx%d %d->%d @%dx%dx%d", w.ks, w.ks, Cin, w.cout, B_, a.H, a.W);
      tick(TC_DIRECT, fl);
      if (o.st) {
        tock();
        DRT_LAUNCH(gn_chan_stats_kernel, dim3(B_ * w.cout), dim3(256), stream_, (const float*)o.p, (const float*)nullptr, w.cout, 0,
                   a.H * a.W, o.st, rag_of(a.H), a.H);
        if (noting()) snprintf(prof_note_, sizeof prof_note_, "gn_chan_stats(direct) C=%d @%dx%dx%d", w.cout, B_, a.H, a.W);
        tick(TC_GN, 4.0 * B_ * (double)w.cout * a.H * a.W, 1);
      }
    }
    return o;
  }

  void launch_fir(const FirArgs& fa, bool up, bool by_level = false) {
    const int H = fa.H, W = fa.W, BC = fa.BC;
    const bool tiled = by_level ? (W % 4 == 0 && dec_W(H) >= 64 && rag_all_mult4(H)) : fir_use_tiled(W);
    if (tiled && !fir_scalar_) {
      if (up) DRT_LAUNCH(fir_up2_tiled_kernel, dim3(((W + 63) / 64) * ((H + 7) / 8), BC), dim3(256), stream_, fa);
      else DRT_LAUNCH(fir_down2_tiled_kernel, dim3(((W / 2 + 63) / 64) * ((H / 2 + 7) / 8), BC), dim3(256), stream_, fa);
    } else {
      if (up) DRT_LAUNCH(fir_up2_kernel, dim3((H * W + 255) / 256, BC), dim3(256), stream_, fa);
      else DRT_LAUNCH(fir_down2_kernel, dim3(((H / 2) * (W / 2) + 255) / 256, BC), dim3(256), stream_, fa);
    }
  }

  Tensor fir(const Tensor& a, bool up, const Xform& xf, Tensor* raw = nullptr) {
    Tensor o = up ? new_tensor(a.C, a.H * 2, a.W * 2) : new_tensor(a.C, a.H / 2, a.W / 2);
    if (raw) {
      *raw = up ? new_tensor(a.C, a.H * 2, a.W * 2) : new_tensor(a.C, a.H / 2, a.W / 2);
      raw->amax = a.amax;
    }
    if (dry_) return o;
    FirArgs fa{a.p, o.p, xf.scale, xf.shift, xf.act, B_ * a.C, a.H, a.W, raw ? raw->p : nullptr, a.C, rag_of(a.H)};
    tock();
    launch_fir(fa, up, true);
    if (noting()) snprintf(prof_note_, sizeof prof_note_, "fir-%s C=%d @%dx%dx%d%s", up ? "up" : "down", a.C, B_, a.H, a.W, raw ? " +raw" : "");
    tick(TC_FIR, 4.0 * B_ * (double)a.C * (a.H * a.W + (raw ? 2.0 : 1.0) * o.H * o.W));
    return o;
  }

  Tensor res_block(const Mod& m, Tensor& a, Tensor* b, const FwdCtl& ctl) {
    const ResW& r = res_.at(m.idx);
    float *sc0, *sh0, *sc1, *sh1;
    const float *bd0, *bd1;
    gn_coeffs(a, b, r.g0w, r.g0b, &sc0, &sh0, &bd0);
    Xform x0{sc0, sh0, 1, bd0};
    const float* temb = ctl.bias_table ? ctl.bias_table + r.temb_off : nullptr;
    Tensor h, xs;
    bool have_xs = false;
    Tensor sh_t; bool sc_side = false;
    auto shortcut_early = [&](const Tensor& sa, const Tensor* sb, int Ch, int Hh) {
      if (!r.has_c2) return;
      const bool fold = runs_on_h2_split3(r.c1, Ch, Hh, dec_W(Hh)) && shortcut_foldable(r.c2, sa, sb) && !((nofold_levels_ >> level_of(Hh)) & 1);
      if (fold || !side_enabled()) return;
      side_begin();
      sh_t = conv(r.c2, sa, sb, Xform{}, r.c2.bias, nullptr, nullptr, 1.f, ctl);
      side_end();
      sc_side = true;
    };
    if (m.up || m.down) {
      SG_REQUIRE(b == nullptr, "resample block with concat input");
      Tensor hr = fir(a, m.up, x0, &xs);
      have_xs = true;
      shortcut_early(xs, nullptr, r.c0.cout, hr.H);
      h = conv(r.c0, hr, nullptr, Xform{nullptr, nullptr, 0, bd0}, nullptr, temb, nullptr, 1.f, ctl, true);
      drop(hr);
    } else {
      shortcut_early(a, b, r.c0.cout, a.H);
      h = conv(r.c0, a, b, x0, nullptr, temb, nullptr, 1.f, ctl, true);
    }
    arena_.release(sc0); arena_.release(sh0);
    gn_coeffs(h, nullptr, r.g1w, r.g1b, &sc1, &sh1, &bd1);
    Xform x1{sc1, sh1, 1, bd1};
    Tensor out;
    const float inv_sqrt2 = 0.70710678118654752440f;
    if (r.has_c2) {
      const Tensor& sa = have_xs ? xs : a;
      const Tensor* sb = have_xs ? nullptr : b;
      if (runs_on_h2_split3(r.c1, h.C, h.H, dec_W(h.H)) && shortcut_foldable(r.c2, sa, sb) && !((nofold_levels_ >> level_of(h.H)) & 1)) {
        const Shortcut scin{&r.c2, &sa, sb};
        out = conv(r.c1, h, nullptr, x1, r.c1.bias, nullptr, nullptr, inv_sqrt2, ctl, true, &scin);
      } else {
        if (sc_side) side_join();
        else sh_t = conv(r.c2, sa, sb, Xform{}, r.c2.bias, nullptr, nullptr, 1.f, ctl);
        out = conv(r.c1, h, nullptr, x1, r.c1.bias, nullptr, sh_t.p, inv_sqrt2, ctl, true);
        drop(sh_t);
      }
    } else {
      SG_REQUIRE(b == nullptr, "identity shortcut with concat input");
      out = conv(r.c1, h, nullptr, x1, r.c1.bias, nullptr, a.p, inv_sqrt2, ctl, true);
    }
    if (have_xs) drop(xs);
    drop(h);
    arena_.release(sc1); arena_.release(sh1);
    return out;
  }

  Tensor attn_block(const Mod& m, Tensor& x, const FwdCtl& ctl) {
    const AttnW& w = attn_.at(m.idx);
    float *sc, *sh;
    gn_coeffs(x, nullptr, w.gw, w.gb, &sc, &sh);
    Tensor qkv = conv(w.qkv, x, nullptr, Xform{sc, sh, 0}, w.qkv.bias, nullptr, nullptr, 1.f, ctl);
    arena_.release(sc); arena_.release(sh);
    Tensor o = new_tensor(x.C, x.H, x.W);
    if (!dry_) {
      AttnArgs aa{qkv.p, o.p, B_, x.C, x.H * x.W, 1.0f / sqrtf((float)x.C), rag_of(x.H), x.H};
      tock();
      SG_REQUIRE(launch_attn_core(aa, stream_), "attention: unsupported channel count");
      if (noting()) snprintf(prof_note_, sizeof prof_note_, "attention C=%d S=%d B=%d", x.C, x.H * x.W, B_);
      tick(TC_ATTN, 4.0 * B_ * (double)x.C * (x.H * x.W) * (double)(x.H * x.W));
    }
    drop(qkv);
    Tensor out = conv(w.proj, o, nullptr, Xform{}, w.proj.bias, nullptr, x.p, 0.70710678118654752440f, ctl, true);
    drop(o);
    return out;
  }

  bool side_enabled() const { return side_stream_on_ && B_ <= side_max_batch_; }
  bool side_active() const { return side_enabled() && !prof_ && !dry_ && !drt::is_emulator(); }
  drt::event_t* side_event() {
    if (side_ev_next_ == side_ev_.size()) { side_ev_.emplace_back(); SG_CHECK(drt::event_create_order(&side_ev_.back())); }
    return &side_ev_[side_ev_next_++];
  }
  void side_begin() {
    SG_REQUIRE(!side_open_, "side stream: nested section");
    side_open_ = true;
    if (!side_enabled()) return;
    if (!side_pending_) arena_.defer_begin();
    if (!side_active()) return;
    if (!side_stream_ready_) { SG_CHECK(drt::stream_create(&side_stream_)); side_stream_ready_ = true; }
    drt::event_t* e = side_event();
    SG_CHECK(drt::event_record(e, stream_));
    SG_CHECK(drt::stream_wait_event(side_stream_, e));
    std::swap(stream_, side_stream_);
    side_swapped_ = true;
  }
  void side_end() {
    SG_REQUIRE(side_open_, "side stream: end without begin");
    side_open_ = false;
    if (!side_enabled()) return;
    side_pending_ = true;
    if (!side_swapped_) return;
    drt::event_t* e = side_event();
    SG_CHECK(drt::event_record(e, stream_));
    std::swap(stream_, side_stream_);
    side_swapped_ = false;
    side_join_ev_ = e;
  }
  void side_join() {
    if (!side_pending_) return;
    side_pending_ = false;
    if (side_join_ev_) { SG_CHECK(drt::stream_wait_event(stream_, side_join_ev_)); side_join_ev_ = nullptr; }
    arena_.defer_end();
  }
  drt::stream_t side_stream_{}; bool side_stream_ready_ = false, side_open_ = false, side_pending_ = false, side_swapped_ = false;
  std::deque<drt::event_t> side_ev_; size_t side_ev_next_ = 0; drt::event_t* side_join_ev_ = nullptr;
  bool side_stream_on_ = true; int side_max_batch_ = 8;

  void run_forward(const float2* x, long long xbs, const float2* y, long long ybs, float2* out, int B, int F, int T,
                   const FwdCtl& ctl_in) {
    side_ev_next_ = 0; side_open_ = side_pending_ = false; side_join_ev_ = nullptr;
    try { run_forward_main(x, xbs, y, ybs, out, B, F, T, ctl_in); }
    catch (...) {
      if (side_swapped_) { std::swap(stream_, side_stream_); side_swapped_ = false; }
      side_open_ = side_pending_ = false; side_join_ev_ = nullptr;
      throw;
    }
  }
  void run_forward_main(const float2* x, long long xbs, const float2* y, long long ybs, float2* out, int B, int F, int T,
                        const FwdCtl& ctl_in) {
    FwdCtl ctl = ctl_in;
    ctl.bias_step = ctl.step_ptr;
    if (!dry_ && ctl.step_ptr && ctl.bias_table && ctl.bias_bstride == 0 && tot_temb_ > 0) {
      DRT_LAUNCH(bias_select_kernel, dim3((tot_temb_ + 255) / 256), dim3(256), stream_, ctl.bias_table, ctl.bias_sstride, ctl.step_ptr,
                 bias_cur_, tot_temb_);
      ctl.bias_table = bias_cur_; ctl.bias_sstride = 0; ctl.bias_step = nullptr;
    }
    B_ = B;
    cur_F_ = F;
    amax_next_ = 0;
    lds_poison_count_ = 0;
    if (!dry_ && poison_ && arena_base_) SG_CHECK(drt::memset_dev(arena_base_, 0xFF, arena_cap_, stream_));
    if (!dry_ && amax_pool_) {
      const int n = amax_slots_ * B * kAmaxSpread;
      DRT_LAUNCH(zero_floats_kernel, dim3((n + 255) / 256), dim3(256), stream_, amax_pool_, n);
    }
    const NetCfg& c = cfg_;
    const int L = c.n_levels;
    size_t mi = 3;
    auto next = [&]() -> const Mod& { SG_REQUIRE(mi < layout_.size(), "layout exhausted"); return layout_[mi++]; };
    const int FT = F * T;
    std::vector<Tensor> hs;
    Tensor xr = new_tensor(4, F, T);
    const bool entry8 = entry_mfma_ && entry8_.packed && layout_[mi].idx == entry8_idx_;
    Tensor xr8{};
    if (entry8) xr8 = new_tensor(entry8_.cin, F, T);
    if (!dry_) { tock(); const WrapCoef wc{ctl.coef, ctl.coef_bstride, ctl.coef_sstride, ctl.step_ptr, ctl.sign};
      DRT_LAUNCH(entry_kernel, dim3((FT + 255) / 256, B), dim3(256), stream_, x, xbs, y, ybs, xr.p, entry8 ? xr8.p : (float*)nullptr,
                 entry8 ? entry8_.cin : 0, FT, wc, rag_of(F), F, ctl.y_plane);
      tick(TC_MISC, (32.0 + (entry8 ? 4.0 * entry8_.cin : 0.0)) * B * FT); }
    {
      const Mod& m = next();
      const ConvW& w = entry8 ? entry8_ : conv_.at(m.idx);
      hs.push_back(conv(w, entry8 ? xr8 : xr, nullptr, Xform{}, w.bias, nullptr, nullptr, 1.f, ctl, true));
      if (entry8) drop(xr8);
    }
    Tensor pyr_in = xr;
    bool pyr_in_is_xr = true;
    for (int l = 0; l < L; ++l) {
      for (int rb = 0; rb < c.num_res_blocks; ++rb) {
        const Mod& m = next();
        Tensor h = res_block(m, hs.back(), nullptr, ctl);
        SG_REQUIRE(cfg_has_attn(c, h.H) == cfg_has_attn(c, c.image_size >> l),
                   "input height does not match the image_size the network was built for (attention placement, ncsnpp.py:308)");
        if (cfg_has_attn(c, h.H)) {
          const Mod& ma = next();
          Tensor h2 = attn_block(ma, h, ctl);
          drop(h);
          h = h2;
        }
        hs.push_back(h);
      }
      if (l != L - 1) {
        const Mod& m = next();
        Tensor h = res_block(m, hs.back(), nullptr, ctl);
        if (c.progressive_input == 1) {
          const Mod& mc = next();
          Tensor np = fir(pyr_in, false, Xform{});
          if (!pyr_in_is_xr) drop(pyr_in);
          pyr_in = np; pyr_in_is_xr = false;
          const ConvW& w = conv_.at(mc.idx);
          Tensor h2 = conv(w, pyr_in, nullptr, Xform{}, w.bias, nullptr, h.p, 1.f, ctl, true);
          drop(h);
          h = h2;
        }
        hs.push_back(h);
      }
    }
    if (!pyr_in_is_xr) drop(pyr_in);
    drop(xr);

    Tensor h = hs.back();
    {
      const Mod& m1 = next(); Tensor a = res_block(m1, h, nullptr, ctl);
      const Mod& m2 = next(); Tensor b2 = attn_block(m2, a, ctl); drop(a);
      const Mod& m3 = next(); h = res_block(m3, b2, nullptr, ctl); drop(b2);
    }
    Tensor pyramid; bool have_pyr = false;
    for (int l = L - 1; l >= 0; --l) {
      for (int rb = 0; rb < c.num_res_blocks + 1; ++rb) {
        const Mod& m = next();
        Tensor skip = hs.back(); hs.pop_back();
        Tensor o = res_block(m, h, &skip, ctl);
        drop(h); drop(skip);
        h = o;
      }
      SG_REQUIRE(cfg_has_attn(c, h.H) == cfg_has_attn(c, c.image_size >> l),
                 "input height does not match the image_size the network was built for (attention placement, ncsnpp.py:354)");
      if (cfg_has_attn(c, h.H)) {
        const Mod& ma = next();
        Tensor h2 = attn_block(ma, h, ctl);
        drop(h); h = h2;
      }
      if (c.progressive == 1) {
        const Mod& mg = next(); const Mod& mc = next();
        side_begin();
        float *sc, *sh;
        const float* bd;
        gn_coeffs(h, nullptr, gn_.at(mg.idx).first, gn_.at(mg.idx).second, &sc, &sh, &bd);
        const ConvW& w = conv_.at(mc.idx);
        Tensor up; bool have_up = false;
        if (have_pyr) { up = fir(pyramid, true, Xform{}); have_up = true; drop(pyramid); }
        pyramid = conv(w, h, nullptr, Xform{sc, sh, 1, bd}, w.bias, nullptr, have_up ? up.p : nullptr, 1.f, ctl);
        have_pyr = true;
        if (have_up) drop(up);
        arena_.release(sc); arena_.release(sh);
        side_end();
      }
      if (l != 0) {
        const Mod& m = next();
        Tensor o = res_block(m, h, nullptr, ctl);
        side_join();
        drop(h); h = o;
      }
    }
    side_join();
    SG_REQUIRE(hs.empty(), "skip stack not empty");
    Tensor h4;
    if (c.progressive == 1) { h4 = pyramid; drop(h); }
    else {
      const Mod& mg = next(); const Mod& mc = next();
      float *sc, *sh;
      const float* bd;
      gn_coeffs(h, nullptr, gn_.at(mg.idx).first, gn_.at(mg.idx).second, &sc, &sh, &bd);
      const ConvW& w = conv_.at(mc.idx);
      h4 = conv(w, h, nullptr, Xform{sc, sh, 1, bd}, w.bias, nullptr, nullptr, 1.f, ctl);
      arena_.release(sc); arena_.release(sh);
      drop(h);
    }
    SG_REQUIRE(mi == layout_.size(), "forward did not consume every module");
    if (!dry_) {
      ExitArgs ea{h4.p, Wp("output_layer.weight"), Wp("output_layer.bias"), ctl.tvals, ctl.t_bstride, ctl.t_sstride, ctl.step_ptr,
                  c.variant == 1 ? 1 : 0, c.scale_by_sigma,
                  WrapCoef{ctl.coef, ctl.coef_bstride, ctl.coef_sstride, ctl.step_ptr, ctl.sign}, x, xbs, out, FT, rag_of(F), F};
      tock();
      DRT_LAUNCH(exit_kernel, dim3((FT + 255) / 256, B), dim3(256), stream_, ea);
      tick(TC_MISC, 24.0 * B * FT);
      check_launch();
    }
    drop(h4);
  }

  struct GraphKey {
    int B, F, T, corr, ncorr, pred, pf; const void* y; const void* noise; float theta; int dps;
    bool operator==(const GraphKey& o) const {
      return B == o.B && F == o.F && T == o.T && corr == o.corr && ncorr == o.ncorr && pred == o.pred && pf == o.pf && y == o.y &&
             noise == o.noise && theta == o.theta && dps == o.dps;
    }
  };
  const unsigned long long* upload_tables(const std::vector<float>& tab, const std::vector<float>& tv, const std::vector<float>& cf,
                                          unsigned long long seed, int B) {
    SG_REQUIRE(B + 1 <= kMaxStreams, "batch too large for the noise-stream table");
    if (!seed_dev_) seed_dev_ = static_cast<unsigned long long*>(dev_alloc((size_t)kMaxStreams * 8));
    const size_t nb_seed = ((size_t)B + 1) * 8, nb_tab = tab.size() * 4, nb_tv = tv.size() * 4, nb_cf = cf.size() * 4;
    const size_t total = nb_seed + nb_tab + nb_tv + nb_cf;
    if (hstage_pending_) { SG_CHECK(drt::event_sync(&hstage_ev_)); hstage_pending_ = false; }
    if (total > hstage_cap_) {
      if (hstage_) drt::free_host(hstage_);
      hstage_cap_ = std::max(total, size_t(1) << 16);
      SG_CHECK(drt::malloc_host(reinterpret_cast<void**>(&hstage_), hstage_cap_));
    }
    unsigned long long* hs = reinterpret_cast<unsigned long long*>(hstage_);
    hs[0] = seed;
    const bool given = (int)streams_next_.size() == B;
    for (int b = 0; b < B; ++b) hs[1 + b] = given ? streams_next_[b] : (unsigned long long)b;
    streams_next_.clear();
    char* q = hstage_ + nb_seed;
    memcpy(q, tab.data(), nb_tab); memcpy(q + nb_tab, tv.data(), nb_tv);
    if (nb_cf) memcpy(q + nb_tab + nb_tv, cf.data(), nb_cf);
    SG_CHECK(drt::memcpy_h2d(seed_dev_, hs, nb_seed, stream_));
    SG_CHECK(drt::memcpy_h2d(step_table_, q, nb_tab, stream_));
    SG_CHECK(drt::memcpy_h2d(tsteps_, q + nb_tab, nb_tv, stream_));
    if (nb_cf) SG_CHECK(drt::memcpy_h2d(coef_table_, q + nb_tab + nb_tv, nb_cf, stream_));
    if (!hstage_ev_init_) { SG_CHECK(drt::event_create(&hstage_ev_)); hstage_ev_init_ = true; }
    SG_CHECK(drt::event_record(&hstage_ev_, stream_));
    hstage_pending_ = true;
    return seed_dev_;
  }
  char* hstage_ = nullptr; size_t hstage_cap_ = 0; drt::event_t hstage_ev_{}; bool hstage_ev_init_ = false, hstage_pending_ = false;
  static constexpr int kMaxStreams = 4096;
  std::vector<unsigned long long> streams_next_;
  unsigned long long* seed_dev_ = nullptr;
  int graph_captures_ = 0;

  int device_;
  drt::stream_t stream_;
  NetCfg cfg_;
  std::vector<Mod> layout_;
  std::map<std::string, const float*> W_;
  float* blob_ = nullptr; size_t blob_elems_ = 0;
  std::map<int, ResW> res_;
  std::map<int, AttnW> attn_;
  std::map<int, ConvW> conv_;
  std::map<int, std::pair<const float*, const float*>> gn_;
  DenseDesc* dense_descs_ = nullptr; int n_dense_ = 0; int tot_temb_ = 0;
  bool weights_ready_ = false;
  std::vector<void*> owned_, wowned_;
  std::map<int, const float2*> twiddles_;

  Arena arena_; char* arena_base_ = nullptr; size_t arena_cap_ = 0;
  bool dry_ = false;
  void read_knobs() {
    auto flag = [](const char* name, bool dflt) { const char* e = getenv(name); return e ? e[0] == '1' : dflt; };
    const char* e = getenv("SGMSE_CONV_SPLIT");
    split_mode_ = e ? atoi(e) : SGMSE_CONV_SPLIT_DEFAULT;
    SG_REQUIRE(split_mode_ >= 0 && split_mode_ <= 2, "SGMSE_CONV_SPLIT must be 0, 1 or 2");
    wino_ = flag("SGMSE_WINO", true);
    rag_prefix_ = flag("SGMSE_RAGGED_PREFIX", true);
    conv_xcd_map_ = flag("SGMSE_CONV_XCD_MAP", true);
    debug_sync_ = flag("SGMSE_DEBUG_SYNC", false);
    prof_dump_ = flag("SGMSE_PROFILE_DUMP", false);
    e = getenv("SGMSE_TILE_MIN_BLOCKS");
    tile_min_blocks_ = e ? atol(e) : 512L;
    e = getenv("SGMSE_SPLIT_MIN_TILES");
    split_min_tiles_ = e ? atol(e) : 8L;
    e = getenv("SGMSE_WINO_MIN_TILES");
    wino_min_tiles_ = e ? atol(e) : 32L;
    fuse_gn_stats_ = flag("SGMSE_FUSE_GN_STATS", true);
    lds_poison_ = flag("SGMSE_POISON_LDS", false);
    e = getenv("SGMSE_POISON_LDS_AT");
    lds_poison_at_ = e ? atoi(e) : -1;
    lds_poison_upto_ = flag("SGMSE_POISON_LDS_UPTO", false);
    side_stream_on_ = flag("SGMSE_SIDE_STREAM", true);
    e = getenv("SGMSE_SIDE_MAX_BATCH");
    side_max_batch_ = e ? atoi(e) : 8;
    e = getenv("SGMSE_NOFOLD_LEVELS");
    nofold_levels_ = e ? atoi(e) : 0;
    poison_ = flag("SGMSE_POISON", false);
  }
  float* amax_pool_ = nullptr; size_t amax_pool_floats_ = 0; int amax_slots_ = 0, amax_next_ = 0;
  float* next_amax() {
    const int i = amax_next_++;
    if (dry_) return reinterpret_cast<float*>(uintptr_t(1) << 43) + (size_t)i * kAmaxSpread;
    SG_REQUIRE(amax_pool_ && i < amax_slots_, "range-bound pool smaller than the forward needs");
    return amax_pool_ + (size_t)i * B_ * kAmaxSpread;
  }
  long tile_min_blocks_ = 512, split_min_tiles_ = 8;
  static constexpr bool coarse_chunked_ = true, fold_shortcut_ = true, coarse_split_ = true, entry_mfma_ = true;
  ConvW entry8_{}; int entry8_idx_ = -1;
  bool poison_ = false, debug_sync_ = false, conv_xcd_map_ = true, rag_prefix_ = true, wino_ = true;
  long wino_min_tiles_ = 32;
  int nofold_levels_ = 0;
  bool lds_poison_ = false, lds_poison_upto_ = false; int lds_poison_at_ = -1, lds_poison_count_ = 0; unsigned* lds_sink_ = nullptr;
  static constexpr long coarse_splitk_div_ = 4, chunk_max_tiles_ = 8;
  int split_mode_ = SGMSE_CONV_SPLIT_DEFAULT;
  bool prof_dump_ = false;
  char prof_note_[160] = {0};
  static constexpr bool fir_scalar_ = false;
  bool fuse_gn_stats_ = true;
  int B_ = 0, shape_B_ = 0, shape_F_ = 0, shape_T_ = 0;
  float2 *sx_ = nullptr, *sxm_ = nullptr, *sscore_ = nullptr, *sy_ = nullptr; size_t samp_n_ = 0;
  int* step_ctr_ = nullptr;
  float *lang_partial_ = nullptr, *lang_scal_ = nullptr;
  float* bias_cur_ = nullptr;
  float *temb_act_ = nullptr, *bias_table_ = nullptr, *step_table_ = nullptr, *tsteps_ = nullptr, *coef_table_ = nullptr; int temb_rows_ = 0;
  drt::graph_t graph_{}; bool graph_valid_ = false; GraphKey graph_key_{};
  int nfe_ = 0;
  bool prof_ = false; std::vector<ProfRec> prof_recs_; size_t prof_used_ = 0; float prof_ms_[TC_COUNT]; double prof_flops_[TC_COUNT]; int prof_n_[TC_COUNT];
};

}
```

### sgmse_amd/ops.py

```python
from __future__ import annotations

from typing import Dict, Optional, Tuple

import torch

from . import _lib

_ctx: Dict[str, "_lib.Context"] = {}


def default_context(device: "torch.device | str | None" = None) -> "_lib.Context":
    if device is None:
        device = "cpu" if _lib.is_emulator() else torch.device("cuda", torch.cuda.current_device())
    key = str(torch.device(device))
    if key not in _ctx:
        _ctx[key] = _lib.Context(device)
    return _ctx[key]


def _f32(t: Optional[torch.Tensor], name: str, dev) -> Optional[torch.Tensor]:
    return None if t is None else _lib.check_tensor(t, name, torch.float32, dev)


def conv2d(x: torch.Tensor, weight: torch.Tensor, bias: Optional[torch.Tensor] = None, *,
           residual: Optional[torch.Tensor] = None, out_scale: float = 1.0, x2: Optional[torch.Tensor] = None,
           in_scale: Optional[torch.Tensor] = None, in_shift: Optional[torch.Tensor] = None, in_act: bool = False,
           force_direct: bool = False, force_split: Optional[str] = None) -> torch.Tensor:
    ctx = default_context(x.device)
    dev = ctx.device
    x = _f32(x, "x", dev); weight = _f32(weight, "weight", dev)
    B, C1, H, W = x.shape
    C2 = 0 if x2 is None else x2.shape[1]
    Cout, Cin, kh, kw = weight.shape
    if kh != kw or kh not in (1, 3):
        raise ValueError("kernel must be 1x1 or 3x3")
    if Cin != C1 + C2:
        raise ValueError(f"weight expects {Cin} input channels, got {C1}+{C2}")
    out = torch.empty((B, Cout, H, W), dtype=torch.float32, device=dev)
    ctx.use_current_stream()
    ctx.check(ctx.lib.sgmse_op_conv2d(ctx.h, x.data_ptr(), weight.data_ptr(), _lib.ptr(_f32(bias, "bias", dev)),
                                      _lib.ptr(_f32(residual, "residual", dev)), out.data_ptr(), B, Cin, Cout, H, W, kh,
                                      float(out_scale), {None: int(force_direct), 'bf16x3': 2, 'fp16x2': 3, 'wino': 4, 'wino4': 5, 'thin': 6, 'wino2d': 7}[force_split], _lib.ptr(_f32(in_scale, "in_scale", dev)),
                                      _lib.ptr(_f32(in_shift, "in_shift", dev)), int(in_act),
                                      _lib.ptr(_f32(x2, "x2", dev)), C2))
    return out


def group_norm(x: torch.Tensor, weight: torch.Tensor, bias: torch.Tensor, *, act: bool = False,
               x2: Optional[torch.Tensor] = None) -> torch.Tensor:
    ctx = default_context(x.device)
    dev = ctx.device
    x = _f32(x, "x", dev)
    B, C1, H, W = x.shape
    C2 = 0 if x2 is None else x2.shape[1]
    C = C1 + C2
    out = torch.empty((B, C, H, W), dtype=torch.float32, device=dev)
    ctx.use_current_stream()
    ctx.check(ctx.lib.sgmse_op_groupnorm(ctx.h, x.data_ptr(), _f32(weight, "weight", dev).data_ptr(),
                                         _f32(bias, "bias", dev).data_ptr(), out.data_ptr(), B, C, H, W, int(act),
                                         _lib.ptr(_f32(x2, "x2", dev)), C2))
    return out


def fir_resample(x: torch.Tensor, up: bool, in_scale: Optional[torch.Tensor] = None, in_shift: Optional[torch.Tensor] = None,
                 in_act: bool = False, return_raw: bool = False):
    ctx = default_context(x.device)
    x = _f32(x, "x", ctx.device)
    B, Cc, H, W = x.shape
    shape = (B, Cc, 2 * H, 2 * W) if up else (B, Cc, H // 2, W // 2)
    out = torch.empty(shape, dtype=torch.float32, device=ctx.device)
    raw = torch.empty(shape, dtype=torch.float32, device=ctx.device) if return_raw else None
    sc = _f32(in_scale, "in_scale", ctx.device)
    sh = _f32(in_shift, "in_shift", ctx.device)
    if (sc is None) != (sh is None) or (sc is not None and (tuple(sc.shape) != (B, Cc) or tuple(sh.shape) != (B, Cc))):
        raise ValueError("in_scale and in_shift must both be given, with shape [B, C]")
    ctx.use_current_stream()
    ctx.check(ctx.lib.sgmse_op_fir(ctx.h, x.data_ptr(), out.data_ptr(), B * Cc, H, W, int(up), _lib.ptr(sc), _lib.ptr(sh),
                                   int(bool(in_act)), _lib.ptr(raw)))
    return (out, raw) if return_raw else out


def upfirdn2d(x: torch.Tensor, kernel: torch.Tensor, up: int = 1, down: int = 1, pad: Tuple[int, int] = (0, 0)) -> torch.Tensor:
    ctx = default_context(x.device)
    code = {torch.float32: 0, torch.float64: 1, torch.float16: 2}.get(x.dtype)
    if code is None:
        raise ValueError(f"upfirdn2d: input dtype {x.dtype} is not supported (float32, float64, float16 -- op/upfirdn2d_kernel.cu:311)")
    if not kernel.dtype.is_floating_point:
        raise ValueError(f"upfirdn2d: kernel dtype {kernel.dtype} is not a floating-point type")
    if kernel.device != x.device:
        raise ValueError(f"upfirdn2d: kernel on {kernel.device}, input on {x.device} (the reference op checks both tensors, upfirdn2d.cpp:15-16)")
    dt = x.dtype
    x = _lib.check_tensor(x, "input", dt, ctx.device); kernel = kernel.to(dtype=dt).contiguous()
    N, Cc, H, W = x.shape
    kh, kw = kernel.shape
    Ho = (H * up + pad[0] + pad[1] - kh) // down + 1
    Wo = (W * up + pad[0] + pad[1] - kw) // down + 1
    out = torch.empty((N, Cc, Ho, Wo), dtype=dt, device=ctx.device)
    ctx.use_current_stream()
    ctx.check(ctx.lib.sgmse_upfirdn2d_dtype(ctx.h, code, x.data_ptr(), kernel.data_ptr(), out.data_ptr(), N * Cc, H, W, kh, kw, up, up,
                                            down, down, pad[0], pad[1], pad[0], pad[1]))
    return out


def attention(qkv: torch.Tensor) -> torch.Tensor:
    ctx = default_context(qkv.device)
    qkv = _f32(qkv, "qkv", ctx.device)
    B, C3, S = qkv.shape
    out = torch.empty((B, C3 // 3, S), dtype=torch.float32, device=ctx.device)
    ctx.use_current_stream()
    ctx.check(ctx.lib.sgmse_op_attention(ctx.h, qkv.data_ptr(), out.data_ptr(), B, C3 // 3, S))
    return out


def stft(sig: torch.Tensor, n_fft: int, hop_length: int, window: torch.Tensor) -> torch.Tensor:
    ctx = default_context(sig.device)
    squeeze = sig.dim() == 1
    s = _f32(sig.reshape(-1, sig.shape[-1]), "sig", ctx.device)
    B, L = s.shape
    K = L // hop_length + 1 if n_fft % 2 == 0 else (L - 1) // hop_length + 1
    out = torch.empty((B, n_fft // 2 + 1, K), dtype=torch.complex64, device=ctx.device)
    ctx.use_current_stream()
    ctx.check(ctx.lib.sgmse_stft(ctx.h, s.data_ptr(), _f32(window, "window", ctx.device).data_ptr(), out.data_ptr(), B, L,
                                 n_fft, hop_length))
    return out[0] if squeeze else out.reshape(*sig.shape[:-1], n_fft // 2 + 1, K)


def istft(spec: torch.Tensor, n_fft: int, hop_length: int, window: torch.Tensor, length: Optional[int] = None) -> torch.Tensor:
    ctx = default_context(spec.device)
    squeeze = spec.dim() == 2
    s = _lib.check_tensor(spec.reshape(-1, spec.shape[-2], spec.shape[-1]), "spec", torch.complex64, ctx.device)
    B, Fq, K = s.shape
    if Fq != n_fft // 2 + 1:
        raise ValueError("spec has the wrong number of frequency bins for n_fft")
    if length is None:
        length = hop_length * (K - 1)
    out = torch.empty((B, length), dtype=torch.float32, device=ctx.device)
    ctx.use_current_stream()
    ctx.check(ctx.lib.sgmse_istft(ctx.h, s.data_ptr(), _f32(window, "window", ctx.device).data_ptr(), out.data_ptr(), B, K,
                                  n_fft, hop_length, length))
    return out[0] if squeeze else out.reshape(*spec.shape[:-2], length)


_XF = {"exponent": 0, "log": 1, "none": 2}


def spec_transform(spec: torch.Tensor, transform_type: str, factor: float, exponent: float, inverse: bool) -> torch.Tensor:
    if transform_type not in _XF:
        raise NotImplementedError(f"transform_type {transform_type!r}")
    ctx = default_context(spec.device)
    s = _lib.check_tensor(spec, "spec", torch.complex64, ctx.device)
    out = torch.empty_like(s)
    ctx.use_current_stream()
    fn = ctx.lib.sgmse_spec_back if inverse else ctx.lib.sgmse_spec_fwd
    ctx.check(fn(ctx.h, s.data_ptr(), out.data_ptr(), s.numel(), _XF[transform_type], float(factor), float(exponent)))
    return out
```

Measured before the change: 5.694 utterances/s.

## Add Winograd F(4,3) conv3x3 kernel and use it on levels up to four

Adds a one-dimensional Winograd F(4,3) 3x3 convolution kernel with fp16x2-split weights packed in six transform taps. It is enabled by default on eligible layers at levels four and below, where width is a multiple of four, and replaces the F(2,3) Winograd path there. The aim is fewer multiplies per output than F(2,3). In exchange the larger transform constants raise numerical error, and shortcut folding is disabled on those layers.

```diff
diff --git a/sgmse_amd/csrc/conv_launch.h b/sgmse_amd/csrc/conv_launch.h
--- a/sgmse_amd/csrc/conv_launch.h
+++ b/sgmse_amd/csrc/conv_launch.h
@@ -4,6 +4,7 @@
 #include "kernels_conv1x1.h"
 #include "kernels_conv_split.h"
 #include "kernels_conv_wino.h"
+#include "kernels_conv_wino43.h"
 #include "kernels_conv_wino2d.h"
 #include "kernels_conv_thin.h"
 
@@ -164,6 +165,29 @@
   }
 }
 
+inline bool conv_wino43_eligible(int C1, int C2, int Cout, int W) {
+  return Cout % 128 == 0 && (C1 + C2) % 16 == 0 && (C2 == 0 || C1 % 16 == 0) && (C1 + C2) <= 512 && W % 4 == 0;
+}
+inline bool conv_wino43_aligned(const ConvArgs& a) {
+  return reinterpret_cast<uintptr_t>(a.src1) % 16 == 0 && (a.src2 == nullptr || reinterpret_cast<uintptr_t>(a.src2) % 16 == 0);
+}
+inline void launch_conv_wino43(const ConvArgs& a, drt::stream_t st, bool rows4, bool trace = false) {
+  const bool act = a.in_scale && a.in_act;
+#ifdef SGMSE_ABLATION_FULL
+  if (trace) { DRT_LAUNCH((conv3x3_wino43_kernel<8, 1, 1>), dim3(conv_grid_tiles(a, 8), a.Cout / 128, 1), dim3(512), st, a); return; }
+#endif
+  (void)trace;
+  if (rows4) {
+    const dim3 grid(conv_grid_tiles(a, 4), a.Cout / 128, 1);
+    if (act) DRT_LAUNCH((conv3x3_wino43_kernel<4, 1>), grid, dim3(512), st, a);
+    else DRT_LAUNCH((conv3x3_wino43_kernel<4, 0>), grid, dim3(512), st, a);
+  } else {
+    const dim3 grid(conv_grid_tiles(a, 8), a.Cout / 128, 1);
+    if (act) DRT_LAUNCH((conv3x3_wino43_kernel<8, 1>), grid, dim3(512), st, a);
+    else DRT_LAUNCH((conv3x3_wino43_kernel<8, 0>), grid, dim3(512), st, a);
+  }
+}
+
 inline void launch_conv_wino2d(const ConvArgs& a, drt::stream_t st, int abl = 0) {
   const dim3 grid(conv_grid_tiles(a, 4), a.Cout / 128, 1);
   const bool act = a.in_scale && a.in_act;
diff --git a/sgmse_amd/csrc/engine.h b/sgmse_amd/csrc/engine.h
--- a/sgmse_amd/csrc/engine.h
+++ b/sgmse_amd/csrc/engine.h
@@ -259,6 +259,8 @@
   int split_mode = 0;
   const float* packed_wino = nullptr;
   const float* wino_scale = nullptr;
+  const float* packed_wino43 = nullptr;
+  const float* wino43_scale = nullptr;
   const float* bias = nullptr;
   int ks = 1, cin = 0, cout = 0, co_t = 0;
 };
@@ -558,6 +560,17 @@
       float* xb = producer_bound(in_scale, in_shift, Cin, bounds, am2, B);
       a.xbound = xb;
       launch_conv_wino2d(a, stream_);
+      SG_CHECK(drt::stream_sync(stream_));
+      free_tmp(const_cast<float*>(pk)); free_tmp(bounds); free_tmp(xb);
+    } else if (force_direct == 8 || force_direct == 9) {
+      SG_REQUIRE(ks == 3 && conv_wino43_eligible(a.C1, C2, Cout, W) && conv_wino43_aligned(a), "op_conv2d: shape is not eligible for the Winograd F(4,3) kernel");
+      const float* pk = pack_wino43(w_oihw, Cin, Cout, false, &a.co_scale);
+      a.w = pk;
+      float* bounds = input_bounds(x, a.C1, x2, C2, B, H * W);
+      const float* am2 = x2 ? bounds + (size_t)B * kAmaxSpread : nullptr;
+      float* xb = producer_bound(in_scale, in_shift, Cin, bounds, am2, B);
+      a.xbound = xb;
+      launch_conv_wino43(a, stream_, force_direct == 9);
       SG_CHECK(drt::stream_sync(stream_));
       free_tmp(const_cast<float*>(pk)); free_tmp(bounds); free_tmp(xb);
     } else if (force_direct == 4 || force_direct == 5) {
@@ -682,9 +695,10 @@
     SG_REQUIRE(pl.mfma, "bench_conv: shape is not MFMA-eligible");
     if (variant >= 0 && (variant & 512)) { pl.rows = 4; variant &= ~512; }
     int ablate = 0, abl_split = 0;
-    bool split_rows4 = false;
+    bool split_rows4 = false, wino43 = false;
     if (variant >= 0) {
       split_rows4 = (variant >> 23) & 1;
+      wino43 = (variant >> 22) & 1;
       abl_split = (variant >> 12) & 1023;
       if (!(variant & (64 | 128))) { ablate = abl_split & 15; abl_split = 0; }
       variant &= 4095;
@@ -695,6 +709,8 @@
     const bool b3 = smode != 0 && !wino && !wino2d;
     SG_REQUIRE(!(wino || wino2d) || (ks == 3 && conv_wino_eligible(Cin, 0, Cout, W)), "bench_conv: shape is not eligible for the Winograd kernel");
     SG_REQUIRE(!b3 || conv_split_eligible(ks, Cin, 0, Cout), "bench_conv: shape is not eligible for the split kernels");
+    wino43 = wino43 && wino;
+    SG_REQUIRE(!wino43 || conv_wino43_eligible(Cin, 0, Cout, W), "bench_conv: shape is not eligible for the Winograd F(4,3) kernel");
     const size_t nx = (size_t)B * Cin * H * W, no = (size_t)B * Cout * H * W, nw = (size_t)Cout * Cin * ks * ks;
     const size_t ne = packed_weight_elems(ks, Cin, Cout, pl.co_t);
     float* x = static_cast<float*>(dev_alloc_tmp(nx * 4));
@@ -731,7 +747,7 @@
       }
     }
     if (wino || wino2d) {
-      pk3 = wino2d ? pack_wino2d(w, Cin, Cout, false, &a.co_scale) : pack_wino(w, Cin, Cout, false, &a.co_scale); a.w = pk3;
+      pk3 = wino2d ? pack_wino2d(w, Cin, Cout, false, &a.co_scale) : wino43 ? pack_wino43(w, Cin, Cout, false, &a.co_scale) : pack_wino(w, Cin, Cout, false, &a.co_scale); a.w = pk3;
       bounds = input_bounds(x, Cin, nullptr, 0, B, H * W);
       xbound = producer_bound(a.in_scale, a.in_shift, Cin, bounds, nullptr, B); a.xbound = xbound;
     }
@@ -744,6 +760,7 @@
     }
     auto go = [&]() {
       if (wino2d) launch_conv_wino2d(a, stream_, abl_split & 63);
+      else if (wino43) launch_conv_wino43(a, stream_, split_rows4, (abl_split & 64) != 0);
       else if (wino) launch_conv_wino(a, stream_, split_rows4, (abl_split & 64) != 0, abl_split & 63);
       else if (b3) launch_conv_split(a, ks, smode, stream_, split_rows4, abl_split);
       else launch_conv_mfma(a, ks, pl, stream_, variant);
@@ -924,7 +941,10 @@
       c.packed_split = pack_split(c.oihw, ks, cin, cout, c.split_mode, true, &c.split_scale);
     }
     if (conv_thin_eligible(ks, cin, 0, cout)) c.packed_thin = pack_thin(c.oihw, cin, cout, true);
-    if (split_mode_ == 2 && wino_ && ks == 3 && conv_wino_eligible(cin, 0, cout, 2)) c.packed_wino = pack_wino(c.oihw, cin, cout, true, &c.wino_scale);
+    if (split_mode_ == 2 && wino_ && ks == 3 && conv_wino_eligible(cin, 0, cout, 2)) {
+      if (wino43_ && conv_wino43_eligible(cin, 0, cout, 4)) c.packed_wino43 = pack_wino43(c.oihw, cin, cout, true, &c.wino43_scale);
+      else c.packed_wino = pack_wino(c.oihw, cin, cout, true, &c.wino_scale);
+    }
     return c;
   }
 
@@ -966,6 +986,20 @@
     DRT_LAUNCH(wino_co_scale_kernel, dim3((unsigned)((cout_pad + 255) / 256)), dim3(256), stream_, oihw, cin, cout, cout_pad, inv, sc);
     PackWinoArgs pa{oihw, pk, cin, cout, frags};
     DRT_LAUNCH(pack_weights_wino_kernel, dim3((unsigned)((frags + 255) / 256)), dim3(256), stream_, pa, (const float*)sc);
+    *scale_out = inv;
+    return reinterpret_cast<const float*>(pk);
+  }
+
+  const float* pack_wino43(const float* oihw, int cin, int cout, bool weight_owned, const float** scale_out) {
+    const size_t frags = packed_wino43_frags(cin, cout);
+    const int cout_pad = (cout + 127) / 128 * 128;
+    const size_t bytes = packed_wino43_bytes(cin, cout) + (size_t)cout_pad * 4;
+    uint32_t* pk = static_cast<uint32_t*>(weight_owned ? dev_alloc_w(bytes) : dev_alloc_tmp(bytes));
+    float* inv = reinterpret_cast<float*>(pk) + frags * 4;
+    float* sc = inv + cout_pad;
+    DRT_LAUNCH(wino43_co_scale_kernel, dim3((unsigned)cout_pad), dim3(64), stream_, oihw, cin, cout, cout_pad, inv, sc);
+    PackWinoArgs pa{oihw, pk, cin, cout, frags};
+    DRT_LAUNCH(pack_weights_wino43_kernel, dim3((unsigned)((frags + 255) / 256)), dim3(256), stream_, pa, (const float*)sc);
     *scale_out = inv;
     return reinterpret_cast<const float*>(pk);
   }
@@ -1280,6 +1314,9 @@
     return w.packed && w.packed_split && w.split_mode == 2 && w.ks == 3 && w.cout > 32 && conv_split_eligible(3, C, 0, w.cout) &&
            (long)((H + 7) / 8) * ((W + 31) / 32) >= split_min_tiles_;
   }
+  bool runs_on_wino43(const ConvW& w, int H) const {
+    return wino_ && w.packed_wino43 && level_of(H) <= 4 && (long)((H + 7) / 8) * ((dec_W(H) + 31) / 32) >= wino_min_tiles_;
+  }
   bool shortcut_foldable(const ConvW& c2, const Tensor& a, const Tensor* b) const {
     return fold_shortcut_ && c2.packed_split && c2.split_mode == 2 && c2.ks == 1 && conv_split_eligible(1, a.C, b ? b->C : 0, c2.cout) &&
            a.amax && (!b || b->amax);
@@ -1314,9 +1351,11 @@
                         tiles8 >= split_min_tiles_ &&
                         (w.split_mode != 2 || (w.ks == 3 ? xf.bound != nullptr
                                                          : (xf.scale == nullptr && a.amax && (!b || b->amax)))));
-    const bool use_wino = use_split && !coarse_split && wino_ && w.packed_wino && w.ks == 3 && w.split_mode == 2 && xf.bound != nullptr &&
-                          conv_wino_eligible(a.C, b ? b->C : 0, w.cout, 2) && level_of(a.H) <= 5 && tiles8 >= wino_min_tiles_;
+    const bool use_wino = use_split && !coarse_split && wino_ && (w.packed_wino || w.packed_wino43) && w.ks == 3 && w.split_mode == 2 && xf.bound != nullptr &&
+                          conv_wino_eligible(a.C, b ? b->C : 0, w.cout, 2) && level_of(a.H) <= (w.packed_wino43 ? 4 : 5) && tiles8 >= wino_min_tiles_;
     SG_REQUIRE(!use_wino || (a.W % 2 == 0 && (!ragged() || rag_all_mult2(a.H))), "conv: odd width on a Winograd level");
+    const bool use_wino43 = use_wino && w.packed_wino43 != nullptr;
+    SG_REQUIRE(!use_wino43 || (a.W % 4 == 0 && (!ragged() || rag_all_mult4(a.H)) && !sc), "conv: width not a multiple of 4 or a folded shortcut on a Winograd F(4,3) level");
     int kchunk = 0, ksplit = 1;
     float* partial = nullptr;
     if (coarse_split) {
@@ -1393,7 +1432,11 @@
       const long nblk8 = (long)B_ * ((a.H + 7) / 8) * ((a.W + 31) / 32) * ((w.cout + 127) / 128);
       const bool rows4 = coarse_split || nblk8 < tile_min_blocks_;
       if (coarse_split) { ca.kchunk_stages = kchunk; ca.partial = partial; }
-      if (use_wino) {
+      if (use_wino43) {
+        ca.w = w.packed_wino43; ca.co_scale = w.wino43_scale; ca.acc_scale = nullptr;
+        SG_REQUIRE(conv_wino43_aligned(ca), "conv: unaligned source on a Winograd F(4,3) level");
+        launch_conv_wino43(ca, stream_, nblk8 < tile_min_blocks_);
+      } else if (use_wino) {
         ca.w = w.packed_wino; ca.co_scale = w.wino_scale; ca.acc_scale = nullptr;
         launch_conv_wino(ca, stream_, nblk8 < tile_min_blocks_);
       } else {
@@ -1403,7 +1446,7 @@
       if (noting()) {
         char scn[24] = "";
         if (sc) snprintf(scn, sizeof scn, " +shortcut(%d)", ca.sc_C1 + ca.sc_C2);
-        snprintf(prof_note_, sizeof prof_note_, "conv3x3-%s %d->%d @%dx%dx%d%s%s%s%s", use_wino ? "wino" : "split", Cin, w.cout, B_, a.H, a.W, res ? " +res" : "",
+        snprintf(prof_note_, sizeof prof_note_, "conv3x3-%s %d->%d @%dx%dx%d%s%s%s%s", use_wino43 ? "wino43" : use_wino ? "wino" : "split", Cin, w.cout, B_, a.H, a.W, res ? " +res" : "",
                  xf.scale ? " +gn" : "", scn, ca.rag_cols ? " existing-tiles" : "");
       }
       tick(w.ks == 3 ? (w.cout >= 128 ? TC_CONV3_BIG : TC_CONV3) : TC_CONV1, fl);
@@ -1473,7 +1516,7 @@
     Tensor sh_t; bool sc_side = false;
     auto shortcut_early = [&](const Tensor& sa, const Tensor* sb, int Ch, int Hh) {
       if (!r.has_c2) return;
-      const bool fold = runs_on_h2_split3(r.c1, Ch, Hh, dec_W(Hh)) && shortcut_foldable(r.c2, sa, sb) && !((nofold_levels_ >> level_of(Hh)) & 1);
+      const bool fold = runs_on_h2_split3(r.c1, Ch, Hh, dec_W(Hh)) && shortcut_foldable(r.c2, sa, sb) && !((nofold_levels_ >> level_of(Hh)) & 1) && !runs_on_wino43(r.c1, Hh);
       if (fold || !side_enabled()) return;
       side_begin();
       sh_t = conv(r.c2, sa, sb, Xform{}, r.c2.bias, nullptr, nullptr, 1.f, ctl);
@@ -1499,7 +1542,7 @@
     if (r.has_c2) {
       const Tensor& sa = have_xs ? xs : a;
       const Tensor* sb = have_xs ? nullptr : b;
-      if (runs_on_h2_split3(r.c1, h.C, h.H, dec_W(h.H)) && shortcut_foldable(r.c2, sa, sb) && !((nofold_levels_ >> level_of(h.H)) & 1)) {
+      if (runs_on_h2_split3(r.c1, h.C, h.H, dec_W(h.H)) && shortcut_foldable(r.c2, sa, sb) && !((nofold_levels_ >> level_of(h.H)) & 1) && !runs_on_wino43(r.c1, h.H)) {
         const Shortcut scin{&r.c2, &sa, sb};
         out = conv(r.c1, h, nullptr, x1, r.c1.bias, nullptr, nullptr, inv_sqrt2, ctl, true, &scin);
       } else {
@@ -1798,6 +1841,7 @@
     split_mode_ = e ? atoi(e) : SGMSE_CONV_SPLIT_DEFAULT;
     SG_REQUIRE(split_mode_ >= 0 && split_mode_ <= 2, "SGMSE_CONV_SPLIT must be 0, 1 or 2");
     wino_ = flag("SGMSE_WINO", true);
+    wino43_ = flag("SGMSE_WINO43", true);
     rag_prefix_ = flag("SGMSE_RAGGED_PREFIX", true);
     conv_xcd_map_ = flag("SGMSE_CONV_XCD_MAP", true);
     debug_sync_ = flag("SGMSE_DEBUG_SYNC", false);
@@ -1830,7 +1874,7 @@
   long tile_min_blocks_ = 512, split_min_tiles_ = 8;
   static constexpr bool coarse_chunked_ = true, fold_shortcut_ = true, coarse_split_ = true, entry_mfma_ = true;
   ConvW entry8_{}; int entry8_idx_ = -1;
-  bool poison_ = false, debug_sync_ = false, conv_xcd_map_ = true, rag_prefix_ = true, wino_ = true;
+  bool poison_ = false, debug_sync_ = false, conv_xcd_map_ = true, rag_prefix_ = true, wino_ = true, wino43_ = true;
   long wino_min_tiles_ = 32;
   int nofold_levels_ = 0;
   bool lds_poison_ = false, lds_poison_upto_ = false; int lds_poison_at_ = -1, lds_poison_count_ = 0; unsigned* lds_sink_ = nullptr;
diff --git a/sgmse_amd/csrc/kernels_conv_wino43.h b/sgmse_amd/csrc/kernels_conv_wino43.h
--- /dev/null
+++ b/sgmse_amd/csrc/kernels_conv_wino43.h
@@ -0,0 +1,439 @@
+#pragma once
+#include "kernels_conv_wino.h"
+
+namespace sgmse {
+
+template <int ROWS_>
+struct Wino43Geom {
+  static constexpr int KC = 16, ROWS = ROWS_, TROWS = ROWS_ + 2, NF = ROWS_ / 4, NK = 6;
+  static constexpr int PV = 25;
+  static constexpr int ROW_V = 8 * PV;
+  static constexpr int STAGE_V = TROWS * ROW_V;
+  static constexpr int NSROW = 4 * TROWS;
+  static constexpr int NPASS = (NSROW + 5) / 6;
+  static constexpr int CO_V = 512;
+  static constexpr int NDIR = ROWS_ == 4 ? 1 : 2;
+  static constexpr int XCH_V = 4 * NDIR * 16 * 64;
+  static constexpr int LDS_V = (2 * STAGE_V + CO_V) > XCH_V ? (2 * STAGE_V + CO_V) : XCH_V;
+  static_assert(NPASS <= 8, "one staging pass per wave");
+};
+
+inline size_t packed_wino43_frags(int cin, int cout) { return (size_t)((cout + 127) / 128) * (cin / 16) * 18 * 2 * 4 * 64; }
+inline size_t packed_wino43_bytes(int cin, int cout) { return packed_wino43_frags(cin, cout) * 16 + (size_t)((cout + 127) / 128) * 128 * 4; }
+
+__device__ __forceinline__ double wino43_u(double g0, double g1, double g2, int k) {
+  return k == 0 ? 0.25 * g0 : k == 1 ? -(g0 + g1 + g2) / 6.0 : k == 2 ? -(g0 - g1 + g2) / 6.0
+       : k == 3 ? g0 / 24.0 + g1 / 12.0 + g2 / 6.0 : k == 4 ? g0 / 24.0 - g1 / 12.0 + g2 / 6.0 : g2;
+}
+__global__ __launch_bounds__(64) void wino43_co_scale_kernel(const float* src, int cin, int cout, int cout_pad, float* inv_scale, float* scale) {
+  const int co = blockIdx.x;
+  if (co >= cout_pad) return;
+  float m = 0.f;
+  if (co < cout) {
+    for (int i = threadIdx.x; i < cin * 3; i += 64) {
+      const float* g = src + ((size_t)co * cin * 3 + i) * 3;
+      m = fmaxf(m, fmaxf(0.25f * fabsf(g[0]), fabsf(g[2])));
+      for (int k = 1; k < 5; ++k) m = fmaxf(m, fabsf((float)wino43_u(g[0], g[1], g[2], k)));
+    }
+  }
+#pragma unroll
+  for (int o = 32; o >= 1; o >>= 1) m = fmaxf(m, __shfl_xor(m, o));
+  if (threadIdx.x == 0) {
+    const float s = co < cout ? h2_weight_scale(m) : 1.f;
+    scale[co] = s; inv_scale[co] = 1.f / s;
+  }
+}
+__global__ __launch_bounds__(256) void pack_weights_wino43_kernel(PackWinoArgs p, const float* co_scale) {
+  const size_t e = (size_t)blockIdx.x * 256 + threadIdx.x;
+  if (e >= p.total) return;
+  const int lane = (int)(e & 63);
+  size_t r = e >> 6;
+  const int cf = (int)(r & 3); r >>= 2;
+  const int split = (int)(r & 1); r >>= 1;
+  const int k = (int)(r % 6); r /= 6;
+  const int dy = (int)(r % 3); r /= 3;
+  const int nst = p.cin / 16;
+  const int st = (int)(r % nst);
+  const int blk = (int)(r / nst);
+  const int co = blk * 128 + cf * 32 + (lane & 31);
+  const int c0 = st * 16 + 8 * (lane >> 5);
+  const double ws = co < p.cout ? (double)co_scale[co] : 1.0;
+  u32x4 o;
+#pragma unroll
+  for (int q = 0; q < 4; ++q) {
+    uint32_t part[2];
+#pragma unroll
+    for (int h = 0; h < 2; ++h) {
+      const int c = c0 + 2 * q + h;
+      double u = 0.0;
+      if (co < p.cout) {
+        const float* g = p.src + (((size_t)co * p.cin + c) * 3 + dy) * 3;
+        u = wino43_u(g[0], g[1], g[2], k);
+      }
+      u *= ws;
+      const uint32_t hi = drt_f32_to_f16((float)u);
+      const uint32_t lo = drt_f32_to_f16((float)(u - (double)drt_f16_to_f32(hi)));
+      part[h] = split ? lo : hi;
+    }
+    o[q] = part[0] | (part[1] << 16);
+  }
+  reinterpret_cast<u32x4*>(p.dst)[e] = o;
+}
+
+template <int ROWS, int ACT, int TRACE = 0>
+__global__ __launch_bounds__(512, 1) void conv3x3_wino43_kernel(ConvArgs p) {
+  using G = Wino43Geom<ROWS>;
+  using T = WinoTile<ROWS>;
+  using S = SplitH2;
+  constexpr int NF = G::NF, PV = G::PV, NS = 2;
+  __shared__ u32x4 s_all[G::LDS_V];
+  u32x4* const s_in0 = s_all;
+  u32x4* const s_in1 = s_all + G::STAGE_V;
+  f32x4* const s_co = reinterpret_cast<f32x4*>(s_all + 2 * G::STAGE_V);
+
+  const int tid = threadIdx.x;
+  const int wave = drt_uniform(tid >> 6), lane = tid & 63, l31 = lane & 31, kg = lane >> 5;
+  const int cf = wave & 3, kh = wave >> 2;
+  unsigned long long* trace = nullptr;
+  if constexpr (TRACE) {
+    if (tid == 0 && p.trace) {
+      trace = p.trace + 32 * (size_t)(blockIdx.y * gridDim.x + blockIdx.x);
+      trace[0] = (unsigned long long)drt_hw_id() | ((unsigned long long)drt_xcc_id() << 32);
+      trace[1] = drt_clock();
+    }
+  }
+  const int Cin = p.C1 + p.C2;
+  const int tiles_xg = (p.W + 31) >> 5;
+  const int tiles_y = (p.H + ROWS - 1) / ROWS;
+  int b, ty, tx;
+  conv_tile_of(p, (int)blockIdx.x, (int)gridDim.x, tiles_xg, tiles_y, b, ty, tx);
+  if (p.rag_w) { if (!conv_ragged_adjust(p, b, tx)) return; }
+  const int H = p.H, W = p.W;
+  const int tiles_x = (W + 31) >> 5;
+  const int co_blk = blockIdx.y;
+  const int x0 = tx * 32, y0 = ty * ROWS;
+  const unsigned HW = (unsigned)H * (unsigned)W;
+
+  float xb_raw = 0.f;
+  if (p.xbound) xb_raw = p.xbound[b * kAmaxSpread + (tid & (kAmaxSpread - 1))];
+  const bool cld = p.in_scale != nullptr && tid < Cin;
+  const float csc = cld ? p.in_scale[b * Cin + (tid < Cin ? tid : 0)] : 1.f;
+  const float csh = cld ? p.in_shift[b * Cin + (tid < Cin ? tid : 0)] : 0.f;
+
+  const int it_sub = lane / 10, it_j = lane - 10 * it_sub;
+  const int it_rr = 6 * wave + it_sub;
+  const bool it_live = it_sub < 6 && it_rr < G::NSROW;
+  const int it_q = it_rr & 3, it_r = it_live ? it_rr >> 2 : 0;
+  const int it_gy = y0 - 1 + it_r, it_gx = x0 - 4 + 4 * it_j;
+  const bool it_ok = it_live && it_gy >= 0 && it_gy < H && it_gx >= 0 && it_gx < W;
+  const unsigned it_boff = ((unsigned)(4 * it_q) * HW + (it_ok ? (unsigned)(it_gy * W + it_gx) : 0u)) * 4u;
+  const int it_woff = ((it_r * 8 + (it_j - 1)) * PV + (it_q >> 1) * NS) * 2 + (it_q & 1);
+  const bool it_wr = it_live && it_j >= 1 && it_j <= 8;
+  const bool it_run = 6 * wave < G::NSROW;
+  float rin[16];
+  auto load_item = [&](int c0) {
+    const bool first = c0 < p.C1;
+    const float* base = first ? p.src1 + ((size_t)b * p.C1 + c0) * HW : p.src2 + ((size_t)b * p.C2 + (c0 - p.C1)) * HW;
+#pragma unroll
+    for (int c = 0; c < 4; ++c) {
+      const float4 v = *reinterpret_cast<const float4*>(reinterpret_cast<const char*>(base + (size_t)c * HW) + it_boff);
+      rin[4 * c] = v.x; rin[4 * c + 1] = v.y; rin[4 * c + 2] = v.z; rin[4 * c + 3] = v.w;
+    }
+  };
+  float V[6][4];
+  auto produce_co = [&](float x, const f32x4& co) -> float {
+    float o = x * co[0] + co[1];
+    if constexpr (ACT == 1) {
+      const float u = x * co[2] + co[3];
+      o = o * __builtin_amdgcn_rcpf(1.0f + drt_exp2(u));
+    }
+    return it_ok ? o : 0.f;
+  };
+  auto stage_chan_co = [&](int c, const f32x4& co) {
+    const float d1 = produce_co(rin[4 * c], co), d2 = produce_co(rin[4 * c + 1], co);
+    const float d3 = produce_co(rin[4 * c + 2], co), d4 = produce_co(rin[4 * c + 3], co);
+    const float d0 = drt_wave_shr1(d4), d5 = drt_wave_shl1(d1);
+    const float a = d4 - d2, bb = d3 - d1;
+    const float c4 = d4 - 4.f * d2, c3 = d3 - 4.f * d1;
+    V[0][c] = 4.f * (d0 - d2) + a;
+    V[1][c] = c4 + c3;
+    V[2][c] = c4 - c3;
+    V[3][c] = a + 2.f * bb;
+    V[4][c] = a - 2.f * bb;
+    V[5][c] = (d5 - d3) - 4.f * bb;
+  };
+  auto flush_item = [&](u32x4* sbuf) {
+    if (it_wr) {
+      uint2* w = reinterpret_cast<uint2*>(sbuf) + it_woff;
+#pragma unroll
+      for (int k = 0; k < 6; ++k) {
+        uint32_t d01[2], d23[2];
+        S::split2(V[k][0], V[k][1], d01);
+        S::split2(V[k][2], V[k][3], d23);
+        w[k * 8] = make_uint2(d01[0], d23[0]);
+        w[k * 8 + 2] = make_uint2(d01[1], d23[1]);
+      }
+    }
+  };
+
+  const int nst = Cin / G::KC;
+  const float* cs_tab = p.co_scale + (size_t)co_blk * 128;
+  float acc_raw[16];
+  conv_acc_raw<T>(p, b, co_blk, cf, kg, acc_raw);
+  auto load_cs = [&](float (&cs)[16]) {
+#pragma unroll
+    for (int r = 0; r < 16; ++r) cs[r] = cs_tab[cf * 32 + 4 * kg + (r & 3) + 8 * (r >> 2)];
+  };
+  if (it_run) load_item(0);
+  float kx = 1.f;
+  if (p.xbound) {
+#pragma unroll
+    for (int o = 32; o >= 1; o >>= 1) xb_raw = fmaxf(xb_raw, __shfl_xor(xb_raw, o));
+    kx = h2_weight_scale(xb_raw) * 0.125f;
+  }
+  const float inv_kx = 1.f / kx;
+  if (tid < Cin) {
+    constexpr float nl2e = -1.4426950408889634f;
+    f32x4 v;
+    v[0] = csc * kx; v[1] = csh * kx; v[2] = csc * nl2e; v[3] = csh * nl2e;
+    s_co[tid] = v;
+  }
+  f32x16 acc[3][NF];
+#pragma unroll
+  for (int kk = 0; kk < 3; ++kk) {
+    float init[16];
+#pragma unroll
+    for (int r = 0; r < 16; ++r) init[r] = 0.f;
+    if (kk == 1 && kh == 0) {
+      float cs_inv[16];
+      load_cs(cs_inv);
+#pragma unroll
+      for (int r = 0; r < 16; ++r) init[r] = acc_raw[r] * (kx / cs_inv[r]);
+    }
+#pragma unroll
+    for (int f = 0; f < NF; ++f)
+#pragma unroll
+      for (int r = 0; r < 16; ++r) acc[kk][f][r] = init[r];
+  }
+
+  const u32x4* wblk = reinterpret_cast<const u32x4*>(p.w) + (size_t)co_blk * nst * 18 * NS * 4 * 64;
+  const unsigned a_boff = (unsigned)((cf * 64 + lane) * 16);
+  auto load_a = [&](int st, int tap, u32x4 (&a)[NS]) {
+    const int dy = tap / 3, k = 3 * kh + (tap - 3 * dy);
+    const u32x4* q = wblk + (size_t)((st * 3 + dy) * 6 + k) * NS * 4 * 64;
+#pragma unroll
+    for (int s = 0; s < NS; ++s) a[s] = *reinterpret_cast<const u32x4*>(reinterpret_cast<const char*>(q + s * 4 * 64) + a_boff);
+  };
+  const int b_lane = l31 * PV + kg * NS;
+
+  u32x4 bq[2][NS];
+  auto compute_tap = [&](const u32x4* sbuf, int tap, const u32x4 (&a)[NS], int phase, bool stage_here, int c0n, u32x4* nxt) {
+    const int dy = tap / 3, kk = tap - 3 * dy;
+    const u32x4* sb = sbuf + b_lane + dy * G::ROW_V + (3 * kh + kk) * 4;
+    f32x4 co2[2];
+    if (phase >= 0 && stage_here) {
+#pragma unroll
+      for (int c = 0; c < 2; ++c) co2[c] = s_co[c0n + 4 * it_q + 2 * phase + c];
+    }
+#pragma unroll
+    for (int s = 0; s < NS; ++s) bq[0][s] = sb[s];
+#pragma unroll
+    for (int f = 0; f < NF; ++f) {
+      if (f + 1 < NF) {
+        const u32x4* q = sb + (f + 1) * 4 * G::ROW_V;
+#pragma unroll
+        for (int s = 0; s < NS; ++s) bq[(f + 1) & 1][s] = q[s];
+      }
+      __builtin_amdgcn_sched_barrier(SGMSE_SPLIT_FENCE);
+#pragma unroll
+      for (int k = 0; k < S::NP; ++k) acc[kk][f] = S::mfma(a[S::pa(k)], bq[f & 1][S::pb(k)], acc[kk][f]);
+      if (phase >= 0 && stage_here) {
+        constexpr int CPF = 2 / NF;
+#pragma unroll
+        for (int c = 0; c < CPF; ++c) stage_chan_co(2 * phase + f * CPF + c, co2[f * CPF + c]);
+        if (phase == 1 && f == NF - 1) flush_item(nxt);
+      }
+      __builtin_amdgcn_sched_barrier(SGMSE_SPLIT_FENCE);
+    }
+  };
+
+  __syncthreads();
+  if (it_run) {
+#pragma unroll
+    for (int c = 0; c < 4; ++c) stage_chan_co(c, s_co[4 * it_q + c]);
+    flush_item(s_in0);
+    load_item((nst > 1 ? 1 : 0) * G::KC);
+  }
+  __syncthreads();
+
+  if constexpr (TRACE) { if (trace) trace[2] = drt_clock(); }
+  constexpr int AR = 3, AD = AR - 1, NTAP = 9;
+  unsigned long long tbar = 0, ttap[NTAP] = {0, 0, 0, 0, 0, 0, 0, 0, 0};
+  const bool tracer = TRACE && p.trace && (tid == 0 || tid == 256);
+  u32x4 ar[AR][NS];
+#pragma unroll
+  for (int t = 0; t < AD; ++t) load_a(0, t, ar[t]);
+#pragma unroll 1
+  for (int st = 0; st < nst; ++st) {
+    const int stn = st + 1 < nst ? st + 1 : st;
+    const int stl = st + 2 < nst ? st + 2 : nst - 1;
+    const u32x4* cur = (st & 1) ? s_in1 : s_in0;
+    u32x4* nxt = (st & 1) ? s_in0 : s_in1;
+#pragma unroll
+    for (int tap = 0; tap < NTAP; ++tap) {
+      unsigned long long tc0 = 0;
+      if constexpr (TRACE) tc0 = drt_clock();
+      const int ntap = (tap + AD) % NTAP;
+      const int nstg = tap + AD < NTAP ? st : stn;
+      load_a(nstg, ntap, ar[(tap + AD) % AR]);
+      __builtin_amdgcn_sched_barrier(0);
+      const bool ca = tap < 2, cb = tap >= NTAP - 2;
+      const int phase = ca ? tap : cb ? tap - (NTAP - 2) : -1;
+      const bool stage_here = phase >= 0 && it_run && (ca ? kh == 0 : kh == 1) && st + 1 < nst;
+      compute_tap(cur, tap, ar[tap % AR], phase, stage_here, stn * G::KC, nxt);
+      if (phase == 1 && stage_here && st + 2 < nst) load_item(stl * G::KC);
+      if constexpr (TRACE) { __builtin_amdgcn_sched_barrier(0); ttap[tap] += drt_clock() - tc0; }
+    }
+    if constexpr (TRACE) {
+      const unsigned long long tb = drt_clock();
+      __syncthreads();
+      tbar += drt_clock() - tb;
+    } else {
+      __syncthreads();
+    }
+  }
+  if constexpr (TRACE) {
+    if (trace) { trace[3] = drt_clock(); trace[6] = tbar; }
+    if (tracer) {
+      unsigned long long* tq = p.trace + 32 * (size_t)(blockIdx.y * gridDim.x + blockIdx.x) + (tid == 0 ? 11 : 21);
+#pragma unroll
+      for (int i = 0; i < NTAP; ++i) tq[i] = ttap[i];
+      tq[NTAP] = tbar;
+    }
+  }
+
+  constexpr bool ALL_TO_A = ROWS == 4;
+  const bool fin_wave = !ALL_TO_A || kh == 0;
+  const int ef = ALL_TO_A ? 0 : kh;
+  int tid_e = (int)threadIdx.x;
+  DRT_PIN_INT(tid_e);
+  const int lane_e = tid_e & 63, l31_e = lane_e & 31, kg_e = lane_e >> 5;
+  const int yy_raw = y0 + 4 * ef + (l31_e >> 3), x = x0 + 4 * (l31_e & 7);
+  const bool okc = x < W;
+  const bool inside = x0 + 32 <= W && y0 + ROWS <= H;
+  const size_t ubase = (size_t)b * p.Cout * HW;
+  const int co_l = co_blk * 128 + cf * 32 + 4 * kg_e;
+  const int yy = yy_raw < H ? yy_raw : H - 1;
+  const unsigned lane_boff = (((unsigned)co_l * (unsigned)H + (unsigned)yy) * (unsigned)W + (unsigned)(okc ? x : 0)) * 4u;
+  auto soff = [&](int r) -> unsigned { return (unsigned)((r & 3) + 8 * (r >> 2)) * HW * 4u; };
+  const drt_buf obuf = drt_make_buf(p.out + ubase), rbuf = drt_make_buf(p.res ? p.res + ubase : p.out);
+  const bool has_res = p.res != nullptr;
+  float2 rr[16][2];
+  if (fin_wave && has_res) {
+#pragma unroll
+    for (int r = 0; r < 16; ++r) { rr[r][0] = drt_buf_load2(rbuf, lane_boff, soff(r)); rr[r][1] = drt_buf_load2(rbuf, lane_boff + 8u, soff(r)); }
+  }
+  if constexpr (TRACE) { if (trace) trace[7] = drt_clock() - trace[3]; }
+  float yv[4][16];
+  {
+    float4* xs = reinterpret_cast<float4*>(s_all);
+    auto slot = [&](int dir, int r) -> float4* { return xs + (((cf * G::NDIR + dir) * 16 + r) * 64 + lane_e); };
+    auto part_a = [&](int f, int r) -> float4 {
+      const float m1 = acc[1][f][r], m2 = acc[2][f][r];
+      const float sp = m1 + m2, sm = m1 - m2;
+      return make_float4(acc[0][f][r] + sp, sm, sp, sm);
+    };
+    auto part_b = [&](int f, int r) -> float4 {
+      const float m3 = acc[0][f][r], m4 = acc[1][f][r];
+      const float s = m3 + m4, t = m3 - m4;
+      return make_float4(s, 2.f * t, 4.f * s, 8.f * t + acc[2][f][r]);
+    };
+    if (kh == 0) {
+      if constexpr (!ALL_TO_A) {
+#pragma unroll
+        for (int r = 0; r < 16; ++r) *slot(1, r) = part_a(NF - 1, r);
+      }
+    } else {
+#pragma unroll
+      for (int r = 0; r < 16; ++r) *slot(0, r) = part_b(0, r);
+    }
+    if constexpr (TRACE) { if (trace) trace[8] = drt_clock() - trace[3]; }
+    __syncthreads();
+    if constexpr (TRACE) { if (trace) trace[9] = drt_clock() - trace[3]; }
+    if (!fin_wave) return;
+    if (kh == 0) {
+#pragma unroll
+      for (int r = 0; r < 16; ++r) {
+        const float4 pb = *slot(0, r), pa = part_a(0, r);
+        yv[0][r] = pa.x + pb.x; yv[1][r] = pa.y + pb.y; yv[2][r] = pa.z + pb.z; yv[3][r] = pa.w + pb.w;
+      }
+    } else {
+      if constexpr (!ALL_TO_A) {
+#pragma unroll
+        for (int r = 0; r < 16; ++r) {
+          const float4 pa = *slot(1, r), pb = part_b(NF - 1, r);
+          yv[0][r] = pa.x + pb.x; yv[1][r] = pa.y + pb.y; yv[2][r] = pa.z + pb.z; yv[3][r] = pa.w + pb.w;
+        }
+      }
+    }
+  }
+  if constexpr (TRACE) { if (trace) trace[5] = drt_clock() - trace[3]; }
+  auto finish = [&](auto guard_tag) {
+    constexpr bool GUARD = decltype(guard_tag)::value;
+    float cs_inv[16];
+    load_cs(cs_inv);
+    float s1[16], s2[16], vmax = 0.f;
+    const bool ok = !GUARD || (okc && yy_raw < H);
+#pragma unroll
+    for (int r = 0; r < 16; ++r) {
+      float v[4];
+#pragma unroll
+      for (int i = 0; i < 4; ++i) v[i] = yv[i][r] * cs_inv[r] * inv_kx;
+      if (has_res) { v[0] += rr[r][0].x; v[1] += rr[r][0].y; v[2] += rr[r][1].x; v[3] += rr[r][1].y; }
+#pragma unroll
+      for (int i = 0; i < 4; ++i) v[i] *= p.out_scale;
+      if (ok) {
+        drt_buf_store2(obuf, make_float2(v[0], v[1]), lane_boff, soff(r));
+        drt_buf_store2(obuf, make_float2(v[2], v[3]), lane_boff + 8u, soff(r));
+      }
+      if (GUARD) {
+#pragma unroll
+        for (int i = 0; i < 4; ++i) v[i] = ok ? v[i] : 0.f;
+      }
+      vmax = fmaxf(fmaxf(vmax, fmaxf(fabsf(v[0]), fabsf(v[1]))), fmaxf(fabsf(v[2]), fabsf(v[3])));
+      s1[r] = (v[0] + v[1]) + (v[2] + v[3]);
+      s2[r] = (v[0] * v[0] + v[1] * v[1]) + (v[2] * v[2] + v[3] * v[3]);
+    }
+    DRT_PIN_HERE(vmax);
+    if constexpr (TRACE) { if (trace) trace[10] = drt_clock() - trace[3]; }
+    if (p.stats_out && y0 + 4 * ef < H) {
+      auto butterfly = [&](float (&sv)[16]) -> float {
+        float a[8];
+#pragma unroll
+        for (int k = 0; k < 8; ++k) a[k] = drt_xadd<16>(sv[k], sv[k + 8]);
+        float c[4];
+#pragma unroll
+        for (int k = 0; k < 4; ++k) c[k] = drt_xadd<8>(a[k], a[k + 4]);
+        const float d0 = drt_xadd<7>(c[0], c[2]), d1 = drt_xadd<7>(c[1], c[3]);
+        return drt_add_xor2(drt_xadd<1>(d0, d1));
+      };
+      const float e2 = butterfly(s2);
+      __builtin_amdgcn_sched_barrier(0);
+      const float e1 = butterfly(s1);
+      const int r = ((l31_e >> 4) & 1) * 8 + ((l31_e >> 3) & 1) * 4 + ((l31_e >> 2) & 1) * 2 + (l31_e & 1);
+      const int co = co_l + (r & 3) + 8 * (r >> 2);
+      float* so = p.stats_out + ((size_t)(b * p.Cout + co) * p.stats_nsub + (size_t)((y0 + 4 * ef) >> 2) * tiles_x + tx) * 2;
+      so[0] = e1; so[1] = e2;
+    }
+    if (p.amax_out) {
+#pragma unroll
+      for (int o = 32; o >= 1; o >>= 1) vmax = fmaxf(vmax, __shfl_xor(vmax, o));
+      if (lane_e == 0) drt_atomic_max_nonneg(p.amax_out + b * kAmaxSpread + ((blockIdx.x * 8 + wave) & (kAmaxSpread - 1)), vmax);
+    }
+    DRT_CODE_MARKER(GUARD);
+  };
+  if (inside) finish(std::false_type{}); else finish(std::true_type{});
+  if constexpr (TRACE) { if (trace) trace[4] = drt_clock(); }
+}
+
+}
diff --git a/sgmse_amd/ops.py b/sgmse_amd/ops.py
--- a/sgmse_amd/ops.py
+++ b/sgmse_amd/ops.py
@@ -40,7 +40,7 @@
     ctx.use_current_stream()
     ctx.check(ctx.lib.sgmse_op_conv2d(ctx.h, x.data_ptr(), weight.data_ptr(), _lib.ptr(_f32(bias, "bias", dev)),
                                       _lib.ptr(_f32(residual, "residual", dev)), out.data_ptr(), B, Cin, Cout, H, W, kh,
-                                      float(out_scale), {None: int(force_direct), 'bf16x3': 2, 'fp16x2': 3, 'wino': 4, 'wino4': 5, 'thin': 6, 'wino2d': 7}[force_split], _lib.ptr(_f32(in_scale, "in_scale", dev)),
+                                      float(out_scale), {None: int(force_direct), 'bf16x3': 2, 'fp16x2': 3, 'wino': 4, 'wino4': 5, 'thin': 6, 'wino2d': 7, 'wino43': 8, 'wino43_4': 9}[force_split], _lib.ptr(_f32(in_scale, "in_scale", dev)),
                                       _lib.ptr(_f32(in_shift, "in_shift", dev)), int(in_act),
                                       _lib.ptr(_f32(x2, "x2", dev)), C2))
     return out
```

Measured after the change: 6.161 utterances/s (median of 6 runs). 8.2% higher.
